# meudnaes/VoronoiRT

Hardware: AMD Instinct MI355X
Metric: formal-solve cell-updates/sec (higher is better)
Workload: dtype f64

## Files before the change

include/voronoirt.h:

```cpp
#ifndef VORONOIRT_H
#define VORONOIRT_H

#include <stdint.h>

#ifdef __cplusplus
extern "C" {
#endif

#define VRT_OK 0
#define VRT_EINVAL (-1)
#define VRT_EGRID (-2)
#define VRT_ENODEVICE (-3)
#define VRT_ENOMEM (-4)
#define VRT_EIO (-5)

typedef struct vrt_grid vrt_grid;
typedef struct vrt_plan vrt_plan;

#define VRT_ALPHA_SITE 0
#define VRT_ALPHA_SITE_LAM 1
#define VRT_ALPHA_ANGLE_SITE_LAM 2
#define VRT_ALPHA_ANGLE_NATIVE 3
#define VRT_ALPHA_SITE_LAM_NATIVE 4

// ... 25 lines not shown
                       int n_sweeps, vrt_plan **out);
void vrt_plan_destroy(vrt_plan *p);
int64_t vrt_plan_num_levels(const vrt_plan *p);
int64_t vrt_plan_num_nodes(const vrt_plan *p);
int vrt_plan_get_upwind(const vrt_plan *p, int64_t angle, int64_t *up, double *dots, double *w,
                        double *r);

int vrt_plan_execute(vrt_plan *p, int64_t nlam, int64_t ld, const double *S, const double *alpha,
                     int alpha_mode, const double *I0_up, const double *I0_down,
                     const double *weights, double *J, double *I_out);
int vrt_plan_execute_dev(vrt_plan *p, int64_t nlam, int64_t ld, const double *dS,
                         const double *dalpha, int alpha_mode, const double *dI0_up,
                         const double *dI0_down, const double *weights_host, double *dJ,
                         double *dI_out, void *stream);
int vrt_grid_get_storage_order(const vrt_grid *g, int dir, int64_t *out);
int64_t vrt_plan_native_alpha_count(const vrt_plan *p, int64_t nlam);
int vrt_plan_native_pair_block(const vrt_plan *p);
int vrt_plan_native_pair_block_f32(const vrt_plan *p);
int vrt_plan_alpha_to_native_dev(vrt_plan *p, int64_t nlam, int64_t ld, const double *dalpha,
                                 double *dalpha_native, void *stream);
int vrt_plan_alpha_to_native_dev_f32(vrt_plan *p, int64_t nlam, int64_t ld, const float *dalpha,
                                     float *dalpha_native, void *stream);

int64_t vrt_plan_native_plane_count(const vrt_plan *p, int64_t nlam);
int vrt_plan_to_native_dev(vrt_plan *p, int64_t nlam, int64_t ld, const double *d_in, double *d_up, double *d_down,
                           void *stream);
int vrt_plan_from_native_dev(vrt_plan *p, int dir, int64_t nlam, int64_t ld, const double *d_native, double *d_out,
                             void *stream);
int vrt_plan_j_from_native_dev(vrt_plan *p, int64_t nlam, int64_t ld, const double *dJ_up, const double *dJ_down,
                               double *dJ, void *stream);
int vrt_plan_execute_native_dev(vrt_plan *p, int64_t nlam, const double *dS_up, const double *dS_down,
                                const double *dalpha, int alpha_mode, const double *dI0_up, const double *dI0_down,
                                const double *weights_host, double *dJ_up, double *dJ_down, void *stream);
int vrt_plan_to_native_dev_f32(vrt_plan *p, int64_t nlam, int64_t ld, const float *d_in, float *d_up, float *d_down,
                               void *stream);
int vrt_plan_from_native_dev_f32(vrt_plan *p, int dir, int64_t nlam, int64_t ld, const float *d_native, float *d_out,
                                 void *stream);
int vrt_plan_j_from_native_dev_f32(vrt_plan *p, int64_t nlam, int64_t ld, const float *dJ_up, const float *dJ_down,
                                   float *dJ, void *stream);
int vrt_plan_execute_native_dev_f32(vrt_plan *p, int64_t nlam, const float *dS_up, const float *dS_down,
                                    const float *dalpha, int alpha_mode, const float *dI0_up, const float *dI0_down,
                                    const double *weights_host, float *dJ_up, float *dJ_down, void *stream);

int vrt_lambda_update_native_dev(vrt_grid *g, int64_t nlam, const double *dJ_up, const double *dJ_down,
                                 const double *dB_up, const double *deps, double *dS_up, double *dS_down,
                                 double *max_rel_change, void *stream);
int vrt_rates_populations_native_dev(vrt_grid *g, int64_t nlam, const double *lambda, const int64_t blocks[6],
                                     const double *dJ_up, const double *dJ_down, const double *planck2,
                                     double lambda0, double c0, const double *d_doppler_width, const double *d_gamma,
                                     double sigma_bb_const, const double *sigma_bf1, const double *sigma_bf2,
                                     const double *d_temperature, const double *d_lte_populations, double hc_over_kB,
                                     double pref_ij, double pref_ji, const double *d_C, const double *d_atom_density,
                                     double *d_R, double *d_populations, void *stream);

int vrt_plan_execute_dev_f32(vrt_plan *p, int64_t nlam, int64_t ld, const float *dS,
                             const float *dalpha, int alpha_mode, const float *dI0_up,
                             const float *dI0_down, const double *weights_host, float *dJ,
                             float *dI_out, void *stream);
int vrt_plan_last_sweep_timing(const vrt_plan *p, double *ms, int64_t *launches);
int vrt_plan_check(vrt_plan *p);
int vrt_plan_last_path(const vrt_plan *p);
int vrt_plan_set_option(vrt_plan *p, const char *name, const char *value);
int vrt_grid_set_option(vrt_grid *g, const char *name, const char *value);

typedef struct vrt_schedule vrt_schedule;
int vrt_schedule_build(const vrt_grid *g, int dir, const int64_t *up, int n_sweeps, vrt_schedule **out);
int64_t vrt_schedule_num_nodes(const vrt_schedule *s);
int64_t vrt_schedule_num_levels(const vrt_schedule *s);
int vrt_schedule_get(const vrt_schedule *s, int64_t *site, int32_t *zflags, int64_t *level_off);
void vrt_schedule_destroy(vrt_schedule *s);
int vrt_layer_schedule(const vrt_grid *g, int dir, const int64_t *up, int n_sweeps, uint32_t *vis,
                       int32_t *nlev, int64_t *n_visits);
int vrt_layer_sorted_slots(const vrt_grid *g, int dir, const uint32_t *vis, int64_t *store, int64_t *self);

typedef struct vrt_patch_schedule vrt_patch_schedule;
int vrt_patch_schedule_build(const vrt_grid *g, int dir, const int64_t *up, int n_sweeps, int own_target,
                             int entry_cap, vrt_patch_schedule **out, int64_t counts[6]);
int vrt_patch_schedule_get(const vrt_patch_schedule *s, int32_t *layer_patch_off, int32_t *patch_own_lo,
                           int32_t *patch_own_cnt, int32_t *patch_nlev, int64_t *patch_ent_off,
                           int32_t *entry_pos, uint32_t *entry_vis, uint32_t *entry_loc);
int vrt_patch_schedule_get_deps(const vrt_patch_schedule *s, int64_t *dep_off, int32_t *dep_list);
int vrt_patch_schedule_get_layers(const vrt_patch_schedule *s, uint32_t *vis, int32_t *nlev, int64_t *n_visits);
void vrt_patch_schedule_destroy(vrt_patch_schedule *s);

int vrt_delaunay_up(vrt_grid *g, const double k[3], const double *S, const double *I0,
                    int64_t nI0, const double *alpha, int n_sweeps, double *I_out);
int vrt_delaunay_down(vrt_grid *g, const double k[3], const double *S, const double *I0,
                      int64_t nI0, const double *alpha, int n_sweeps, double *I_out);

#define VRT_METRIC_EUCLIDEAN   0
#define VRT_METRIC_PERIODIC_XY 1
#define VRT_RASTER_NEAREST     1
#define VRT_RASTER_INV_DIST2   2
int vrt_grid_nearest(vrt_grid *g, int64_t nq, const double *q_zxy, int metric, int k, int64_t *idx, double *dist);
int vrt_grid_to_raster_dev(vrt_grid *g, int64_t nz, int64_t nx, int64_t ny, const double *z, const double *x,
                           const double *y, int metric, int mode, int64_t nf, int64_t ld, const double *d_fields,
                           double *d_raster, void *stream);
int vrt_raster_to_grid_dev(vrt_grid *g, int64_t nz, int64_t nx, int64_t ny, const double *z, const double *x,
                           const double *y, int64_t nf, const double *d_raster, int64_t ld, double *d_fields,
                           void *stream);
int vrt_grid_to_raster(vrt_grid *g, int64_t nz, int64_t nx, int64_t ny, const double *z, const double *x,
                       const double *y, int metric, int mode, int64_t nf, int64_t ld, const double *fields,
                       double *raster);
int vrt_raster_to_grid(vrt_grid *g, int64_t nz, int64_t nx, int64_t ny, const double *z, const double *x,
                       const double *y, int64_t nf, const double *raster, int64_t ld, double *fields);
int vrt_grid_raster_stats(const vrt_grid *g, double *nearest_ms, double *gather_ms, int64_t *queries,
                          int64_t *walk_steps, int64_t *fallbacks);

int vrt_sample_sites(int device, int64_t nz, int64_t nx, int64_t ny, const double *z, const double *x, const double *y,
                     const double *quantity, int64_t n_sites, uint64_t seed, int64_t batch, int64_t max_proposals,
                     double *pos_zxy, int64_t *proposals_used);
int vrt_sample_sites_dev(int device, int64_t nz, int64_t nx, int64_t ny, const double *z, const double *x,
                         const double *y, const double *d_quantity, int64_t n_sites, uint64_t seed, int64_t batch,
                         int64_t max_proposals, double *d_pos_zxy, int64_t *proposals_used, void *stream);

int vrt_lambda_update_dev(vrt_grid *g, int64_t nlam, int64_t ld, const double *dJ, const double *dB,
                          const double *deps, const double *dS_old, double *dS_new,
                          double *max_rel_change, void *stream);

int vrt_line_opacity_dev(vrt_plan *p, int64_t nlam, const double *lambda, double lambda0, double c0,
                         const double *d_velocity, const double *d_doppler_width, const double *d_gamma,
                         const double *d_line_strength, const double *d_alpha_cont, double *d_alpha_native,
                         void *stream);
int vrt_line_opacity_dev_f32(vrt_plan *p, int64_t nlam, const double *lambda, double lambda0, double c0,
                             const double *d_velocity, const double *d_doppler_width, const double *d_gamma,
                             const double *d_line_strength, const double *d_alpha_cont, float *d_alpha_native,
                             void *stream);

int vrt_plan_execute_line(vrt_plan *p, int64_t nlam, int64_t ld, const double *lambda, double lambda0, double c0,
                          const double *velocity, const double *doppler_width, const double *gamma,
                          const double *line_strength, const double *alpha_cont, const double *S, const double *I0_up,
                          const double *I0_down, const double *weights, double *J);

int vrt_line_terms_dev(vrt_grid *g, const double *d_gamma_static, const double *d_gamma_unsold,
                       const double *d_populations, double strength_const, double Bij, double Bji, double *d_gamma,
                       double *d_line_strength, void *stream);

typedef struct vrt_lambda vrt_lambda;
typedef struct vrt_line_case {
    int64_t nlam;
    const double *lambda;
    int64_t blocks[6];
    double lambda0, c0;
    const double *velocity;
    const double *doppler_width;
    const double *gamma_static;
    const double *gamma_unsold;
    const double *alpha_cont;
    const double *eps;
    const double *temperature;
    const double *atom_density;
    const double *B0;
    const double *lte_populations;
    const double *C;
    const double *planck2;
    const double *sigma_bf1, *sigma_bf2;
    double strength_const, Bij, Bji;
    double sigma_bb_const, hc_over_kB, pref_ij, pref_ji;
} vrt_line_case;
int vrt_lambda_create(vrt_plan *p, const vrt_line_case *lc, const double *weights, vrt_lambda **out);
int vrt_lambda_iterate(vrt_lambda *s, double *max_rel_change);
int vrt_lambda_get(vrt_lambda *s, double *J, double *S, double *populations, double *R, double *gamma);
void vrt_lambda_destroy(vrt_lambda *s);

typedef struct vrt_multi vrt_multi;
int vrt_multi_create(int n_devices, const int *devices, int64_t n, const double *pos_zxy, const int64_t *nbr, int64_t D1,
// ... 80 lines not shown
```

voronoirt_amd/_lib.py:

```python
from __future__ import annotations

import ctypes
import os

HERE = os.path.dirname(os.path.abspath(__file__))
LIB_PATH = os.path.join(HERE, "libvrt_hip.so")
if os.environ.get("VRT_LIB_PATH"):
    LIB_PATH = os.environ["VRT_LIB_PATH"]

c_i64 = ctypes.c_int64
c_dbl = ctypes.c_double
p_i64 = ctypes.POINTER(ctypes.c_int64)
p_i32 = ctypes.POINTER(ctypes.c_int32)
p_dbl = ctypes.POINTER(ctypes.c_double)
p_int = ctypes.POINTER(ctypes.c_int)
vp = ctypes.c_void_p

VRT_OK, VRT_EINVAL, VRT_EGRID, VRT_ENODEVICE, VRT_ENOMEM, VRT_EIO = 0, -1, -2, -3, -4, -5
ALPHA_SITE, ALPHA_SITE_LAM, ALPHA_ANGLE_SITE_LAM, ALPHA_ANGLE_NATIVE, ALPHA_SITE_LAM_NATIVE = 0, 1, 2, 3, 4
METRIC_EUCLIDEAN, METRIC_PERIODIC_XY = 0, 1
RASTER_NEAREST, RASTER_INV_DIST2 = 1, 2

class LineCaseStruct(ctypes.Structure):
    _fields_ = [("nlam", c_i64), ("lambda_", p_dbl), ("blocks", c_i64 * 6), ("lambda0", c_dbl), ("c0", c_dbl),
# ... 20 lines not shown
    "vrt_grid_num_layer_offsets": (c_i64, [vp, ctypes.c_int]),
    "vrt_grid_get_layers": (ctypes.c_int, [vp, ctypes.c_int, p_i64]),
    "vrt_grid_get_perm": (ctypes.c_int, [vp, ctypes.c_int, p_i64]),
    "vrt_grid_get_delaunay_lines": (ctypes.c_int, [vp, p_dbl]),
    "vrt_direction": (None, [c_dbl, c_dbl, p_dbl]),
    "vrt_plan_create": (ctypes.c_int, [vp, c_i64, p_dbl, ctypes.c_int, ctypes.POINTER(vp)]),
    "vrt_plan_create_ex": (ctypes.c_int, [vp, c_i64, p_dbl, p_int, ctypes.c_int,
                                          ctypes.POINTER(vp)]),
    "vrt_plan_destroy": (None, [vp]),
    "vrt_plan_num_levels": (c_i64, [vp]),
    "vrt_plan_num_nodes": (c_i64, [vp]),
    "vrt_plan_get_upwind": (ctypes.c_int, [vp, c_i64, p_i64, p_dbl, p_dbl, p_dbl]),
    "vrt_plan_execute": (ctypes.c_int, [vp, c_i64, c_i64, p_dbl, p_dbl, ctypes.c_int, p_dbl, p_dbl,
                                        p_dbl, p_dbl, p_dbl]),
    "vrt_plan_execute_dev": (ctypes.c_int, [vp, c_i64, c_i64, vp, vp, ctypes.c_int, vp, vp, p_dbl,
                                            vp, vp, vp]),
    "vrt_plan_execute_dev_f32": (ctypes.c_int, [vp, c_i64, c_i64, vp, vp, ctypes.c_int, vp, vp, p_dbl,
                                                vp, vp, vp]),
    "vrt_plan_native_plane_count": (c_i64, [vp, c_i64]),
    "vrt_plan_to_native_dev": (ctypes.c_int, [vp, c_i64, c_i64, vp, vp, vp, vp]),
    "vrt_plan_from_native_dev": (ctypes.c_int, [vp, ctypes.c_int, c_i64, c_i64, vp, vp, vp]),
    "vrt_plan_j_from_native_dev": (ctypes.c_int, [vp, c_i64, c_i64, vp, vp, vp, vp]),
    "vrt_plan_execute_native_dev": (ctypes.c_int, [vp, c_i64, vp, vp, vp, ctypes.c_int, vp, vp, p_dbl, vp, vp, vp]),
    "vrt_plan_to_native_dev_f32": (ctypes.c_int, [vp, c_i64, c_i64, vp, vp, vp, vp]),
    "vrt_plan_from_native_dev_f32": (ctypes.c_int, [vp, ctypes.c_int, c_i64, c_i64, vp, vp, vp]),
    "vrt_plan_j_from_native_dev_f32": (ctypes.c_int, [vp, c_i64, c_i64, vp, vp, vp, vp]),
    "vrt_plan_execute_native_dev_f32": (ctypes.c_int, [vp, c_i64, vp, vp, vp, ctypes.c_int, vp, vp, p_dbl, vp, vp, vp]),
    "vrt_plan_check": (ctypes.c_int, [vp]),
    "vrt_lambda_update_native_dev": (ctypes.c_int, [vp, c_i64, vp, vp, vp, vp, vp, vp, p_dbl, vp]),
    "vrt_rates_populations_native_dev": (ctypes.c_int, [vp, c_i64, p_dbl, p_i64, vp, vp, p_dbl, c_dbl, c_dbl, vp, vp,
                                                        c_dbl, p_dbl, p_dbl, vp, vp, c_dbl, c_dbl, c_dbl, vp, vp, vp,
                                                        vp, vp]),
    "vrt_grid_get_storage_order": (ctypes.c_int, [vp, ctypes.c_int, p_i64]),
    "vrt_plan_native_alpha_count": (c_i64, [vp, c_i64]),
    "vrt_plan_native_pair_block": (ctypes.c_int, [vp]),
    "vrt_plan_native_pair_block_f32": (ctypes.c_int, [vp]),
    "vrt_plan_alpha_to_native_dev": (ctypes.c_int, [vp, c_i64, c_i64, vp, vp, vp]),
    "vrt_line_opacity_dev": (ctypes.c_int, [vp, c_i64, p_dbl, c_dbl, c_dbl, vp, vp, vp, vp, vp, vp, vp]),
    "vrt_line_opacity_dev_f32": (ctypes.c_int, [vp, c_i64, p_dbl, c_dbl, c_dbl, vp, vp, vp, vp, vp, vp, vp]),
    "vrt_plan_alpha_to_native_dev_f32": (ctypes.c_int, [vp, c_i64, c_i64, vp, vp, vp]),
    "vrt_plan_execute_line": (ctypes.c_int, [vp, c_i64, c_i64, p_dbl, c_dbl, c_dbl, p_dbl, p_dbl, p_dbl, p_dbl, p_dbl,
                                             p_dbl, p_dbl, p_dbl, p_dbl, p_dbl]),
    "vrt_line_terms_dev": (ctypes.c_int, [vp, vp, vp, vp, c_dbl, c_dbl, c_dbl, vp, vp, vp]),
    "vrt_lambda_create": (ctypes.c_int, [vp, ctypes.POINTER(LineCaseStruct), p_dbl, ctypes.POINTER(vp)]),
    "vrt_lambda_iterate": (ctypes.c_int, [vp, p_dbl]),
    "vrt_lambda_get": (ctypes.c_int, [vp, p_dbl, p_dbl, p_dbl, p_dbl, p_dbl]),
    "vrt_lambda_destroy": (None, [vp]),
    "vrt_multi_create": (ctypes.c_int, [ctypes.c_int, p_int, c_i64, p_dbl, p_i64, c_i64, p_dbl, c_i64, p_dbl, p_int,
                                        ctypes.c_int, ctypes.POINTER(vp)]),
    "vrt_multi_execute": (ctypes.c_int, [vp, c_i64, c_i64, p_dbl, p_dbl, ctypes.c_int, p_dbl, p_dbl, p_dbl, p_dbl]),
    "vrt_multi_set_shard": (ctypes.c_int, [vp, ctypes.c_char_p]),
    "vrt_multi_last_shard": (ctypes.c_int, [vp]),
    "vrt_multi_uses_rccl": (ctypes.c_int, [vp]),
    "vrt_multi_destroy": (None, [vp]),
    "vrt_multi_execute_line": (ctypes.c_int, [vp, c_i64, c_i64, p_dbl, c_dbl, c_dbl, p_dbl, p_dbl, p_dbl, p_dbl, p_dbl, p_dbl,
                                              p_dbl, p_dbl, p_dbl, p_dbl]),
    "vrt_multi_lambda_create": (ctypes.c_int, [vp, ctypes.POINTER(LineCaseStruct), p_dbl, ctypes.POINTER(vp)]),
    "vrt_multi_lambda_iterate": (ctypes.c_int, [vp, p_dbl]),
    "vrt_multi_lambda_get": (ctypes.c_int, [vp, p_dbl, p_dbl, p_dbl, p_dbl, p_dbl]),
    "vrt_multi_lambda_destroy": (None, [vp]),
    "vrt_rates_populations_dev": (ctypes.c_int, [vp, c_i64, c_i64, p_dbl, p_i64, vp, p_dbl, c_dbl, c_dbl, vp, vp,
                                                 c_dbl, p_dbl, p_dbl, vp, vp, c_dbl, c_dbl, c_dbl, vp, vp, vp,
                                                 vp, vp]),
    "vrt_plan_last_sweep_timing": (ctypes.c_int, [vp, p_dbl, p_i64]),
    "vrt_plan_last_path": (ctypes.c_int, [vp]),
    "vrt_plan_set_option": (ctypes.c_int, [vp, ctypes.c_char_p, ctypes.c_char_p]),
    "vrt_grid_set_option": (ctypes.c_int, [vp, ctypes.c_char_p, ctypes.c_char_p]),
    "vrt_schedule_build": (ctypes.c_int, [vp, ctypes.c_int, p_i64, ctypes.c_int,
                                          ctypes.POINTER(vp)]),
    "vrt_schedule_num_nodes": (c_i64, [vp]),
    "vrt_schedule_num_levels": (c_i64, [vp]),
    "vrt_schedule_get": (ctypes.c_int, [vp, p_i64, p_i32, p_i64]),
    "vrt_schedule_destroy": (None, [vp]),
    "vrt_layer_schedule": (ctypes.c_int, [vp, ctypes.c_int, p_i64, ctypes.c_int,
                                          ctypes.POINTER(ctypes.c_uint32), p_i32, p_i64]),
    "vrt_layer_sorted_slots": (ctypes.c_int, [vp, ctypes.c_int, ctypes.POINTER(ctypes.c_uint32), p_i64, p_i64]),
    "vrt_patch_schedule_build": (ctypes.c_int, [vp, ctypes.c_int, p_i64, ctypes.c_int, ctypes.c_int, ctypes.c_int,
                                                ctypes.POINTER(vp), p_i64]),
    "vrt_patch_schedule_get": (ctypes.c_int, [vp, p_i32, p_i32, p_i32, p_i32, p_i64, p_i32,
                                              ctypes.POINTER(ctypes.c_uint32), ctypes.POINTER(ctypes.c_uint32)]),
    "vrt_patch_schedule_get_deps": (ctypes.c_int, [vp, p_i64, p_i32]),
    "vrt_patch_schedule_get_layers": (ctypes.c_int, [vp, ctypes.POINTER(ctypes.c_uint32), p_i32, p_i64]),
    "vrt_patch_schedule_destroy": (None, [vp]),
    "vrt_lambda_update_dev": (ctypes.c_int, [vp, c_i64, c_i64, vp, vp, vp, vp, vp, p_dbl, vp]),
    "vrt_short_characteristics": (ctypes.c_int, [c_i64, c_i64, c_i64, p_dbl, p_dbl, p_dbl, c_i64, p_dbl,
                                                 p_int, p_dbl, c_i64, p_dbl, c_i64, p_dbl, ctypes.c_int,
                                                 ctypes.c_int, p_dbl]),
    "vrt_regular_create": (ctypes.c_int, [c_i64, c_i64, c_i64, p_dbl, p_dbl, p_dbl, ctypes.c_int,
                                          ctypes.POINTER(vp)]),
    "vrt_regular_destroy": (None, [vp]),
    "vrt_regular_execute_dev": (ctypes.c_int, [vp, c_i64, p_dbl, p_int, vp, c_i64, vp, c_i64, c_i64, vp,
                                               ctypes.c_int, vp, vp]),
    "vrt_regular_last_solve_ms": (ctypes.c_int, [vp, p_dbl]),
    "vrt_regular_execute_line": (ctypes.c_int, [vp, c_i64, p_dbl, p_int, p_dbl, c_i64, p_dbl, c_dbl, c_dbl, p_dbl, p_dbl,
                                                p_dbl, p_dbl, p_dbl, p_dbl, p_dbl, ctypes.c_int, p_dbl]),
    "vrt_regular_lambda_create": (ctypes.c_int, [vp, c_i64, p_dbl, p_int, p_dbl, ctypes.POINTER(LineCaseStruct), ctypes.c_int,
                                                 ctypes.POINTER(vp)]),
    "vrt_regular_lambda_iterate": (ctypes.c_int, [vp, p_dbl]),
    "vrt_regular_lambda_get": (ctypes.c_int, [vp, p_dbl, p_dbl, p_dbl, p_dbl, p_dbl]),
    "vrt_regular_lambda_destroy": (None, [vp]),
    "vrt_synth_opacity_dev": (ctypes.c_int, [c_i64, c_i64, c_i64, p_dbl, c_i64, p_dbl, p_dbl, c_dbl, c_dbl, c_dbl, c_dbl,
                                             c_dbl, c_dbl, c_dbl, c_dbl, vp, vp, vp, vp, vp, vp, vp, vp, vp, vp]),
    "vrt_synth_opacity": (ctypes.c_int, [ctypes.c_int, c_i64, c_i64, c_i64, p_dbl, c_i64, p_dbl, p_dbl, c_dbl, c_dbl,
                                         c_dbl, c_dbl, c_dbl, c_dbl, c_dbl, c_dbl, p_dbl, p_dbl, p_dbl, p_dbl, p_dbl,
                                         p_dbl, p_dbl, p_dbl, p_dbl]),
    "vrt_regular_emergent_dev": (ctypes.c_int, [vp, p_dbl, c_i64, vp, vp, ctypes.c_int, vp, vp]),
    "vrt_top_intensity": (ctypes.c_int, [c_i64, c_i64, c_i64, p_dbl, p_dbl, p_dbl, p_dbl, c_i64, p_dbl, p_dbl,
                                         ctypes.c_int, ctypes.c_int, p_dbl]),
    "vrt_tau_unity_dev": (ctypes.c_int, [c_i64, c_i64, c_i64, p_dbl, p_dbl, p_dbl, p_dbl, c_i64, vp, vp, vp]),
    "vrt_tau_unity": (ctypes.c_int, [c_i64, c_i64, c_i64, p_dbl, p_dbl, p_dbl, p_dbl, c_i64, p_dbl, ctypes.c_int,
                                     p_dbl]),
    "vrt_grid_nearest": (ctypes.c_int, [vp, c_i64, p_dbl, ctypes.c_int, ctypes.c_int, p_i64, p_dbl]),
    "vrt_grid_to_raster_dev": (ctypes.c_int, [vp, c_i64, c_i64, c_i64, p_dbl, p_dbl, p_dbl, ctypes.c_int, ctypes.c_int,
                                              c_i64, c_i64, vp, vp, vp]),
    "vrt_raster_to_grid_dev": (ctypes.c_int, [vp, c_i64, c_i64, c_i64, p_dbl, p_dbl, p_dbl, c_i64, vp, c_i64, vp, vp]),
    "vrt_grid_to_raster": (ctypes.c_int, [vp, c_i64, c_i64, c_i64, p_dbl, p_dbl, p_dbl, ctypes.c_int, ctypes.c_int,
                                          c_i64, c_i64, p_dbl, p_dbl]),
    "vrt_raster_to_grid": (ctypes.c_int, [vp, c_i64, c_i64, c_i64, p_dbl, p_dbl, p_dbl, c_i64, p_dbl, c_i64, p_dbl]),
    "vrt_grid_raster_stats": (ctypes.c_int, [vp, p_dbl, p_dbl, p_i64, p_i64, p_i64]),
    "vrt_sample_sites": (ctypes.c_int, [ctypes.c_int, c_i64, c_i64, c_i64, p_dbl, p_dbl, p_dbl, p_dbl, c_i64,
                                        ctypes.c_uint64, c_i64, c_i64, p_dbl, p_i64]),
    "vrt_sample_sites_dev": (ctypes.c_int, [ctypes.c_int, c_i64, c_i64, c_i64, p_dbl, p_dbl, p_dbl, vp, c_i64,
                                            ctypes.c_uint64, c_i64, c_i64, vp, p_i64, vp]),
    "vrt_delaunay_up": (ctypes.c_int, [vp, p_dbl, p_dbl, p_dbl, c_i64, p_dbl, ctypes.c_int, p_dbl]),
    "vrt_delaunay_down": (ctypes.c_int, [vp, p_dbl, p_dbl, p_dbl, c_i64, p_dbl, ctypes.c_int, p_dbl]),
}


class VrtError(RuntimeError):
    def __init__(self, code: int, message: str):
        super().__init__(f"libvrt_hip error {code}: {message}")
        self.code = code
        self.message = message


_lib = None


def load() -> ctypes.CDLL:
    global _lib
    if _lib is not None:
        return _lib
    if not os.path.exists(LIB_PATH):
        raise ImportError(
            f"{LIB_PATH} is missing: build it with `python -m voronoirt_amd.build` "
            "(hipcc --offload-arch=gfx950).  voronoirt_amd has no CPU fallback.")
    if os.environ.get("VRT_NO_TORCH") != "1":
        try:
            import torch
        except Exception:
            pass
    lib = ctypes.CDLL(LIB_PATH)
    for name, (res, args) in PROTOTYPES.items():
        fn = getattr(lib, name)
        fn.restype = res
        fn.argtypes = args
    _lib = lib
    return lib


def check(rc: int) -> None:
    if rc != 0:
        msg = load().vrt_last_error()
        raise VrtError(rc, msg.decode() if msg else "")
```

voronoirt_amd/csrc/vrt_api.cpp:

```cpp
#include <algorithm>
#include <atomic>
#include <chrono>
#include <cmath>
#include <cstdio>
#include <cstdlib>
#include <cstring>
#include <memory>
#include <new>
#include <thread>

#include "vrt_internal.h"

namespace vrt {

static thread_local std::string g_err;

void set_error(const std::string &msg) { g_err = msg; }
int fail(int code, const std::string &msg)
{
    g_err = msg;
    return code;
}

void tuning_from_env(Tuning &t)
{
    static const char *names[] = {"VRT_PATH", "VRT_STEP_K", "VRT_STEP_SINGLE", "VRT_STEP_PAIRS", "VRT_STEP_XCD",
                                  "VRT_STEP_STREAMS", "VRT_STEP_LEVEL_MAP", "VRT_STEP_GROUP_DIR", "VRT_TILE_WIDE",
                                  "VRT_TILE_PRE", "VRT_PATCH_K", "VRT_PATCH_NT", "VRT_PATCH_OWN",
                                  "VRT_PATCH_Q", "VRT_PATCH_TARGET", "VRT_PATCH_SPLIT", "VRT_PAIR_BLOCK", "VRT_PATCH_QUAD", "VRT_PATCH_LEAN", "VRT_PATCH_CHAIN", "VRT_CHAIN_PAIRS", "VRT_CHAIN_SPIN", "VRT_CHAIN_DATAFLAG", "VRT_CHAIN_STATIC", "VRT_LAMBDA_NATIVE", "VRT_DEBUG_FLAGS", "VRT_DEBUG_SKIP_LEVELS",
                                  "VRT_TILE_DEBUG"};
    for (const char *nm : names) {
        const char *e = std::getenv(nm);
        if (e && *e && tuning_set(t, nm, e, false) != VRT_OK) {
            static std::mutex mu;
            static std::vector<std::string> said;
            std::lock_guard<std::mutex> lock(mu);
            if (std::find(said.begin(), said.end(), std::string(nm)) == said.end()) {
                said.push_back(nm);
                std::fprintf(stderr, "[libvrt_hip] ignoring %s=%s: %s\n", nm, e, g_err.c_str());
            }
        }
    }
}

int tuning_set(Tuning &t, const char *name, const char *value, bool created)
{
    if (!name || !value) return fail(VRT_EINVAL, "NULL option name or value");
    const std::string nm(name), v(value);
    if (nm == "VRT_PATH") {
        static const char *paths[] = {"auto", "levels", "tiles", "steps", "patches"};
        for (int i = 0; i < 5; i++)
            if (v == paths[i]) { t.path = i; return VRT_OK; }
        if (v.empty()) { t.path = 0; return VRT_OK; }
        return fail(VRT_EINVAL, "VRT_PATH must be auto, levels, tiles, steps or patches");
    }
    char *end = nullptr;
    const long x = std::strtol(value, &end, 10);
    if (end == value || *end != 0) return fail(VRT_EINVAL, "option " + nm + " needs an integer value");
    struct { const char *name; int *field; long lo, hi; bool creation_only; } tab[] = {
        {"VRT_STEP_K", &t.step_K, 0, 18, false}, {"VRT_STEP_SINGLE", &t.step_single, 0, 1, false},
        {"VRT_STEP_PAIRS", &t.step_pairs, 0, 64, false}, {"VRT_STEP_XCD", &t.step_xcd, 0, 2, false},
        {"VRT_STEP_STREAMS", &t.step_streams, 1, 4, false}, {"VRT_STEP_LEVEL_MAP", &t.step_level_map, 0, 1, false},
        {"VRT_STEP_GROUP_DIR", &t.step_group_dir, 0, 1, false}, {"VRT_TILE_WIDE", &t.tile_wide, 0, 1, false},
        {"VRT_TILE_PRE", &t.tile_pre, 0, 1, false},
        {"VRT_PATCH_K", &t.patch_K, 1, 8, true}, {"VRT_PATCH_NT", &t.patch_NT, 64, 1024, true},
        {"VRT_PATCH_OWN", &t.patch_own, 0, 65535, true}, {"VRT_PATCH_Q", &t.patch_Q, 1, 4, false},
        {"VRT_PATCH_TARGET", &t.patch_target, 0, 1 << 20, false}, {"VRT_PATCH_SPLIT", &t.patch_split, 0, 4096, false}, {"VRT_PAIR_BLOCK", &t.pair_block, 1, 16, true},
        {"VRT_PATCH_QUAD", &t.patch_quad, 0, 1, true}, {"VRT_PATCH_LEAN", &t.patch_lean, 0, 1, false},
        {"VRT_PATCH_CHAIN", &t.patch_chain, 0, 2, false}, {"VRT_CHAIN_PAIRS", &t.chain_pairs, 1, 256, false},
        {"VRT_CHAIN_SPIN", &t.chain_spin, 1, 1 << 20, false}, {"VRT_CHAIN_DATAFLAG", &t.chain_dataflag, 0, 2, false},
        {"VRT_LAMBDA_NATIVE", &t.lambda_native, 0, 1, false}, {"VRT_CHAIN_STATIC", &t.chain_static, 0, 1, false}, {"VRT_DEBUG_FLAGS", &t.debug_flags, 0, 1 << 20, false},
        {"VRT_DEBUG_SKIP_LEVELS", &t.debug_skip_levels, 0, 1, false}, {"VRT_TILE_DEBUG", &t.tile_debug, 0, 1, false},
    };
    for (auto &o : tab)
        if (nm == o.name) {
            if (o.creation_only && created)
                return fail(VRT_EINVAL, "option " + nm + " shapes what plan creation builds: preset it in the environment");
            if (x < o.lo || x > o.hi) return fail(VRT_EINVAL, "option " + nm + " out of range");
            *o.field = (int)x;
            return VRT_OK;
        }
    return fail(VRT_EINVAL, "unknown option " + nm);
}

int use_device(int device)
{
    if (device < 0)
        return fail(VRT_ENODEVICE, "host-only grid handle (device < 0): no compute without a HIP device");
    int cnt = 0;
    hipError_t e = hipGetDeviceCount(&cnt);
    if (e != hipSuccess || cnt <= 0)
        return fail(VRT_ENODEVICE, "no HIP device available (libvrt_hip has no CPU fallback)");
    if (device < 0 || device >= cnt) return fail(VRT_EINVAL, "device ordinal out of range");
    VRT_HIP_TRY(hipSetDevice(device));
    (void)hipGetLastError();
    return VRT_OK;
}

int use_current_device()
{
    int cnt = 0;
    if (hipGetDeviceCount(&cnt) != hipSuccess || cnt <= 0)
        return fail(VRT_ENODEVICE, "no HIP device available (libvrt_hip has no CPU fallback)");
    (void)hipGetLastError();
    return VRT_OK;
}

static void free_grid(vrt_grid *g)
{
    if (!g) return;
    for (PlanCacheEntry *c : g->cache) {
        vrt_plan_destroy(c->plan);
        delete c;
    }
    g->cache.clear();
    raster_locator_free(g);
    dev_free(g->d_pos);
    dev_free(g->d_rowptr);
    dev_free(g->d_col);
    dev_free(g->d_lz);
    dev_free(g->d_lx);
    dev_free(g->d_ly);
    dev_free(g->up.d_order);
    dev_free(g->down.d_order);
    dev_free(g->up.d_rank);
    dev_free(g->down.d_rank);
    dev_free(g->up.d_lay);
    dev_free(g->down.d_lay);
    dev_free(g->d_scalars);
    dev_free(g->d_small);
    if (g->small_ev) (void)hipEventDestroy(g->small_ev);
    if (g->small_copy_ev) (void)hipEventDestroy(g->small_copy_ev);
    if (g->h_small) (void)hipHostFree(g->h_small);
    dev_free(g->up.d_store);
    dev_free(g->down.d_store);
    dev_free(g->up.d_srank);
    dev_free(g->down.d_srank);
    if (g->stream) (void)hipStreamDestroy(g->stream);
    delete g;
}

static int upload_grid(vrt_grid *g)
{
    const int64_t n = g->n;
    const size_t nnz = g->col.size();
    int rc;
    if ((rc = dev_alloc(&g->d_pos, (size_t)3 * n))) return rc;
    if ((rc = dev_alloc(&g->d_rowptr, (size_t)n + 1))) return rc;
    if ((rc = dev_alloc(&g->d_col, nnz))) return rc;
    if ((rc = dev_alloc(&g->d_lz, nnz))) return rc;
// ... 9 lines not shown
        std::vector<int32_t> order((size_t)n);
        for (int64_t i = 0; i < n; i++) order[(size_t)i] = (int32_t)(dir.perm[(size_t)i] - 1);
        if ((rc = dev_alloc(&dir.d_order, (size_t)n))) return rc;
        VRT_HIP_TRY(hipMemcpy(dir.d_order, order.data(), sizeof(int32_t) * n, hipMemcpyHostToDevice));
        std::vector<int32_t> rank((size_t)n);
        for (int64_t i = 0; i < n; i++) rank[(size_t)order[(size_t)i]] = (int32_t)i;
        if ((rc = dev_alloc(&dir.d_rank, (size_t)n))) return rc;
        VRT_HIP_TRY(hipMemcpy(dir.d_rank, rank.data(), sizeof(int32_t) * n, hipMemcpyHostToDevice));
        std::vector<int32_t> srank((size_t)n);
        for (int64_t i = 0; i < n; i++) srank[(size_t)dir.store[(size_t)i]] = (int32_t)i;
        if ((rc = dev_alloc(&dir.d_store, (size_t)n))) return rc;
        if ((rc = dev_alloc(&dir.d_srank, (size_t)n))) return rc;
        VRT_HIP_TRY(hipMemcpy(dir.d_store, dir.store.data(), sizeof(int32_t) * n, hipMemcpyHostToDevice));
        VRT_HIP_TRY(hipMemcpy(dir.d_srank, srank.data(), sizeof(int32_t) * n, hipMemcpyHostToDevice));
        std::vector<int32_t> lay(dir.reduced.size());
        for (size_t j = 0; j < lay.size(); j++) lay[j] = (int32_t)(dir.reduced[j] - 1);
        if ((rc = dev_alloc(&dir.d_lay, lay.size()))) return rc;
        VRT_HIP_TRY(hipMemcpy(dir.d_lay, lay.data(), sizeof(int32_t) * lay.size(), hipMemcpyHostToDevice));
    }
    if ((rc = launch_delaunay_lines(g))) return rc;
    VRT_HIP_TRY(hipStreamSynchronize(g->stream));
    return VRT_OK;
}

static int grid_create_impl(int64_t n, const double *pos, const int64_t *nbr, int64_t D1,
                            const double bounds[6], int device, vrt_grid **out)
{
    if (!out) return fail(VRT_EINVAL, "out is NULL");
    *out = nullptr;
    if (!pos || !nbr || !bounds) return fail(VRT_EINVAL, "NULL argument");
    int rc = device >= 0 ? use_device(device) : VRT_OK;
    if (rc) return rc;
    vrt_grid *g = new (std::nothrow) vrt_grid();
    if (!g) return fail(VRT_ENOMEM, "out of host memory");
    g->device = device;
    rc = build_grid_host(g, n, pos, nbr, D1, bounds);
    if (!rc && device >= 0) rc = upload_grid(g);
    if (rc) {
        free_grid(g);
        return rc;
    }
    *out = g;
    return VRT_OK;
}

static const Direction &direction_of(const vrt_grid *g, int dir) { return dir > 0 ? g->up : g->down; }

static void free_plan(vrt_plan *p)
{
    if (!p) return;
    dev_free(p->d_up1);
    dev_free(p->d_up2);
    dev_free(p->d_d1);
    dev_free(p->d_d2);
    dev_free(p->d_w1);
    dev_free(p->d_w2);
    dev_free(p->d_r1);
    dev_free(p->d_r2);
    dev_free(p->d_node_site);
    dev_free(p->d_node_meta);
    dev_free(p->d_node_u1);
    dev_free(p->d_node_u2);
    dev_free(p->d_angles_up);
    dev_free(p->d_angles_down);
    dev_free(p->d_I);
    for (int i = 0; i < 6; i++) dev_free(p->d_stage[i]);
    dev_free(p->t_u1); dev_free(p->t_u2);
    dev_free(p->t_w1); dev_free(p->t_w2); dev_free(p->t_r1); dev_free(p->t_r2);
    dev_free(p->t_vis);
    dev_free(p->t_loc);
    dev_free(p->t_self);
    dev_free(p->t_vis_s);
    dev_free(p->t_loc_s);
    dev_free(p->t_gpos);
    dev_free(p->t_rank_s);
    dev_free(p->t_loc_ss);
    dev_free(p->t_code_ss);
    dev_free(p->d_nlev); dev_free(p->d_angle_dir); dev_free(p->d_task_map);
    for (int d = 0; d < 2; d++) { dev_free(p->ws_S[d]); dev_free(p->ws_A[d]); dev_free(p->ws_J[d]); }
    dev_free(p->ws_AA);
    for (int i = 0; i < 2; i++) dev_free(p->ws_cg[i]);
    dev_free(p->d_step_angles);
    dev_free(p->d_level_map);
    dev_free(p->d_patch_work);
    dev_free(p->d_chain_items); dev_free(p->d_chain_deps); dev_free(p->d_chain_progress); dev_free(p->d_chain_ctrl);
    for (auto &cs : p->chain_cache) { dev_free(cs.items); dev_free(cs.deps); }
    p->chain_cache.clear();
    if (p->h_chain_status) { (void)hipHostFree(p->h_chain_status); p->h_chain_status = nullptr; }
    if (p->d_chain_dev) { (void)hipFree(p->d_chain_dev); p->d_chain_dev = nullptr; }
    if (p->h_chain_dev_pinned) { (void)hipHostFree(p->h_chain_dev_pinned); p->h_chain_dev_pinned = nullptr; }
    if (p->chain_dev_ev) (void)hipEventDestroy(p->chain_dev_ev);
    dev_free(p->e_pos); dev_free(p->e_u1); dev_free(p->e_u2); dev_free(p->e_vis); dev_free(p->e_loc);
    dev_free(p->e_w1); dev_free(p->e_w2); dev_free(p->e_r1); dev_free(p->e_r2);
    if (p->step_fork) (void)hipEventDestroy(p->step_fork);
    for (int i = 0; i < 4; i++) {
        if (p->step_join[i]) (void)hipEventDestroy(p->step_join[i]);
        if (p->step_stream[i]) (void)hipStreamDestroy(p->step_stream[i]);
    }
    for (CopyLane &l : p->copy_lanes) {
        for (int b = 0; b < 2; b++) {
            if (l.pin[b]) (void)hipHostFree(l.pin[b]);
            if (l.ev[b]) (void)hipEventDestroy(l.ev[b]);
        }
        if (l.st) (void)hipStreamDestroy(l.st);
    }
    if (p->copy_done) (void)hipEventDestroy(p->copy_done);
    if (p->ev0) (void)hipEventDestroy(p->ev0);
    if (p->ev1) (void)hipEventDestroy(p->ev1);
    delete p;
}

static int ensure_level_schedule(vrt_plan *p)
{
    if (p->level_ready) return VRT_OK;
    vrt_grid *g = p->g;
    const int64_t n = g->n;
    const int A = p->A;
    const int n_sweeps = p->n_sweeps;
    std::vector<AngleSchedule> sched((size_t)A);
    {
        unsigned hw = std::thread::hardware_concurrency();
        int nthr = (int)std::min<unsigned>(hw ? hw : 4, 16);
        nthr = std::max(1, std::min(nthr, std::max(A, 1)));
        if (!run_workers(nthr, [&](int t) {
                for (int a = t; a < A; a += nthr) {
                    const bool up = p->dir_of_active[(size_t)a] > 0;
                    build_angle_schedule(up ? g->up : g->down, up, n, n_sweeps,
                                         p->h_up1.data() + (size_t)a * n, p->h_up2.data() + (size_t)a * n,
                                         sched[(size_t)a]);
                }
            }))
            return fail(VRT_ENOMEM, "out of host memory while building the level schedule");
    }
    int64_t max_levels = 0, total = 0;
    for (int a = 0; a < A; a++) {
        if (sched[(size_t)a].bad_site >= 0) return fail(VRT_EGRID, "site without an upwind neighbour");
        max_levels = std::max<int64_t>(max_levels, (int64_t)sched[(size_t)a].level_off.size() - 1);
        total += (int64_t)sched[(size_t)a].site.size();
    }
    std::vector<int32_t> srank_up((size_t)n);
    for (int64_t i = 0; i < n; i++) srank_up[(size_t)g->up.store[(size_t)i]] = (int32_t)i;
    std::vector<uint32_t> node_site((size_t)total), node_meta((size_t)total);
    std::vector<int32_t> node_u1((size_t)total), node_u2((size_t)total);
    p->level_off.assign((size_t)max_levels + 1, 0);
    int64_t at = 0;
    for (int64_t t = 0; t < max_levels; t++) {
        p->level_off[(size_t)t] = at;
        for (int a = 0; a < A; a++) {
            const AngleSchedule &s = sched[(size_t)a];
            if (t + 1 >= (int64_t)s.level_off.size()) continue;
            const int64_t x0 = s.level_off[(size_t)t], x1 = s.level_off[(size_t)t + 1];
            std::vector<std::pair<int32_t, int64_t>> keyed((size_t)(x1 - x0));
            for (int64_t x = x0; x < x1; x++)
                keyed[(size_t)(x - x0)] = {srank_up[(size_t)s.site[(size_t)x]], x};
            std::sort(keyed.begin(), keyed.end());
            for (const auto &kv : keyed) {
                const int64_t x = kv.second;
                node_site[(size_t)at] = s.site[(size_t)x];
                node_meta[(size_t)at] = (uint32_t)a | ((uint32_t)s.zflags[(size_t)x] << 8);
                node_u1[(size_t)at] = p->h_up1[(size_t)a * (size_t)n + s.site[(size_t)x]];
                node_u2[(size_t)at] = p->h_up2[(size_t)a * (size_t)n + s.site[(size_t)x]];
                at++;
            }
        }
    }
    p->level_off[(size_t)max_levels] = at;
    p->n_nodes = total;
// ... 773 lines not shown
        return VRT_OK;
    });
}

struct vrt_patch_schedule {
    vrt::PatchSchedule s;
    vrt::LayerSchedule layers;
};

int vrt_patch_schedule_build(const vrt_grid *g, int dir, const int64_t *up, int n_sweeps, int own_target,
                             int entry_cap, vrt_patch_schedule **out, int64_t counts[6])
{
    if (!g || !up || !out || !counts) return fail(VRT_EINVAL, "NULL argument");
    if (n_sweeps < 1 || own_target < 1 || entry_cap < 1 || entry_cap > 65535)
        return fail(VRT_EINVAL, "need n_sweeps >= 1, own_target >= 1 and 1 <= entry_cap <= 65535");
    *out = nullptr;
    return guarded([&] {
        const int64_t n = g->n;
        std::vector<int32_t> u1((size_t)n), u2((size_t)n);
        for (int64_t i = 0; i < n; i++) {
            const int64_t a = up[2 * i], b = up[2 * i + 1];
            if (a > n || b > n) return fail(VRT_EINVAL, "upwind id out of range");
            u1[(size_t)i] = a >= 1 ? (int32_t)(a - 1) : kNoUpwind;
            u2[(size_t)i] = b >= 1 ? (int32_t)(b - 1) : kNoUpwind;
        }
        std::unique_ptr<vrt_patch_schedule> ps(new vrt_patch_schedule());
        int threads = (int)std::max(1u, std::min(8u, std::thread::hardware_concurrency()));
        if (const char *e = std::getenv("VRT_HOST_THREADS")) threads = std::max(1, std::min(64, std::atoi(e)));
        build_patch_schedule(direction_of(g, dir), dir > 0, n, n_sweeps, u1.data(), u2.data(), own_target, entry_cap,
                             ps->s, threads, &ps->layers);
        if (ps->s.bad_site >= 0)
            return fail(VRT_EGRID, "site " + std::to_string(ps->s.bad_site + 1) + " has no upwind neighbour");
        if (!ps->s.ok) return fail(VRT_EINVAL, "schedule does not fit the packed patch encoding");
        counts[0] = (int64_t)ps->s.patch_own_lo.size();
        counts[1] = (int64_t)ps->s.entry_pos.size();
        counts[2] = ps->s.n_visits;
        counts[3] = ps->s.n_live;
        counts[4] = ps->s.max_entries;
        counts[5] = (int64_t)ps->s.layer_patch_off.size();
        *out = ps.release();
        return VRT_OK;
    });
}

int vrt_patch_schedule_get(const vrt_patch_schedule *s, int32_t *layer_patch_off, int32_t *patch_own_lo,
                           int32_t *patch_own_cnt, int32_t *patch_nlev, int64_t *patch_ent_off,
                           int32_t *entry_pos, uint32_t *entry_vis, uint32_t *entry_loc)
{
    if (!s) return fail(VRT_EINVAL, "NULL schedule");
    const PatchSchedule &p = s->s;
    if (layer_patch_off) std::copy(p.layer_patch_off.begin(), p.layer_patch_off.end(), layer_patch_off);
    if (patch_own_lo) std::copy(p.patch_own_lo.begin(), p.patch_own_lo.end(), patch_own_lo);
    if (patch_own_cnt) std::copy(p.patch_own_cnt.begin(), p.patch_own_cnt.end(), patch_own_cnt);
    if (patch_nlev) std::copy(p.patch_nlev.begin(), p.patch_nlev.end(), patch_nlev);
    if (patch_ent_off) std::copy(p.patch_ent_off.begin(), p.patch_ent_off.end(), patch_ent_off);
    if (entry_pos) std::copy(p.entry_pos.begin(), p.entry_pos.end(), entry_pos);
    if (entry_vis) std::copy(p.entry_vis.begin(), p.entry_vis.end(), entry_vis);
    if (entry_loc) std::copy(p.entry_loc.begin(), p.entry_loc.end(), entry_loc);
    return VRT_OK;
}

int vrt_patch_schedule_get_deps(const vrt_patch_schedule *s, int64_t *dep_off, int32_t *dep_list)
{
    if (!s) return fail(VRT_EINVAL, "NULL schedule");
    const PatchSchedule &p = s->s;
    if (dep_off) std::copy(p.dep_off.begin(), p.dep_off.end(), dep_off);
    if (dep_list) std::copy(p.dep_list.begin(), p.dep_list.end(), dep_list);
    return VRT_OK;
}

int vrt_patch_schedule_get_layers(const vrt_patch_schedule *s, uint32_t *vis, int32_t *nlev, int64_t *n_visits)
{
    if (!s) return fail(VRT_EINVAL, "NULL schedule");
    const LayerSchedule &ls = s->layers;
    if (!ls.ok) return fail(VRT_EINVAL, "schedule does not fit the packed layer-tile encoding");
    if (vis) std::copy(ls.vis.begin(), ls.vis.end(), vis);
    if (nlev) std::copy(ls.nlev.begin(), ls.nlev.end(), nlev);
    if (n_visits) *n_visits = ls.n_visits;
    return VRT_OK;
}

void vrt_patch_schedule_destroy(vrt_patch_schedule *s) { delete s; }

int vrt_grid_get_storage_order(const vrt_grid *g, int dir, int64_t *out)
{
    if (!g || !out) return fail(VRT_EINVAL, "NULL argument");
    const Direction &d = direction_of(g, dir);
    for (int64_t i = 0; i < g->n; i++) out[i] = (int64_t)d.store[(size_t)i] + 1;
    return VRT_OK;
}

int vrt_plan_native_pair_block(const vrt_plan *p) { return p ? 1 << native_lg(p, false) : 0; }
int vrt_plan_native_pair_block_f32(const vrt_plan *p) { return p ? 1 << native_lg(p, true) : 0; }

int64_t vrt_plan_native_alpha_count(const vrt_plan *p, int64_t nlam)
{
    if (!p || nlam < 1) return 0;
    return (int64_t)p->A * ((nlam + 1) / 2 * 2) * p->g->n;
}

static int alpha_native_call(vrt_plan *p, int64_t nlam, int64_t ld, const void *dalpha, void *dalpha_native, void *stream,
                             bool f32)
{
    return guarded([&] {
        if (!p || !dalpha || !dalpha_native) return fail(VRT_EINVAL, "NULL argument");
        if (nlam < 1 || ld < nlam) return fail(VRT_EINVAL, "need nlam >= 1 and ld >= nlam");
        if (p->A != (int)p->n_angles_user)
            return fail(VRT_EINVAL, "per-angle alpha needs every angle active (no θ = 90 direction)");
        std::lock_guard<std::mutex> lock(p->mu);
        int rc = use_device(p->g->device);
        return rc ? rc : alpha_to_native(p, nlam, ld, dalpha, dalpha_native, (hipStream_t)stream, f32);
    });
}

int vrt_plan_alpha_to_native_dev(vrt_plan *p, int64_t nlam, int64_t ld, const double *dalpha,
                                 double *dalpha_native, void *stream)
{
    return alpha_native_call(p, nlam, ld, dalpha, dalpha_native, stream, false);
}

int vrt_plan_alpha_to_native_dev_f32(vrt_plan *p, int64_t nlam, int64_t ld, const float *dalpha, float *dalpha_native,
                                     void *stream)
{
    return alpha_native_call(p, nlam, ld, dalpha, dalpha_native, stream, true);
}

int vrt_plan_execute_dev(vrt_plan *p, int64_t nlam, int64_t ld, const double *dS,
                         const double *dalpha, int alpha_mode, const double *dI0_up,
                         const double *dI0_down, const double *weights_host, double *dJ,
                         double *dI_out, void *stream)
{
    return execute_call(p, caller_args(nlam, ld, dS, dalpha, alpha_mode, dI0_up, dI0_down, weights_host, dJ, dI_out,
                                       (hipStream_t)stream, false));
}

int64_t vrt_plan_native_plane_count(const vrt_plan *p, int64_t nlam)
{
    if (!p || nlam < 1) return 0;
    return ((nlam + 1) / 2 * 2) * p->g->n;
}

int vrt_plan_to_native_dev(vrt_plan *p, int64_t nlam, int64_t ld, const double *d_in, double *d_up, double *d_down, void *stream)
{
    return native_call(p, nlam, ld, d_in && (d_up || d_down), false,
                       [&] { return planes_to_native(p, nlam, ld, d_in, d_up, d_down, (hipStream_t)stream); });
}

int vrt_plan_from_native_dev(vrt_plan *p, int dir, int64_t nlam, int64_t ld, const double *d_native, double *d_out, void *stream)
{
    return native_call(p, nlam, ld, d_native && d_out, false,
                       [&] { return plane_from_native(p, dir > 0 ? 0 : 1, nlam, ld, d_native, d_out, (hipStream_t)stream); });
}

int vrt_plan_j_from_native_dev(vrt_plan *p, int64_t nlam, int64_t ld, const double *dJ_up, const double *dJ_down, double *dJ,
                               void *stream)
{
    return native_call(p, nlam, ld, dJ && (dJ_up || dJ_down), false,
                       [&] { return J_from_native(p, nlam, ld, dJ_up, dJ_down, dJ, (hipStream_t)stream); });
}

int vrt_plan_execute_native_dev(vrt_plan *p, int64_t nlam, const double *dS_up, const double *dS_down, const double *dalpha,
                                int alpha_mode, const double *dI0_up, const double *dI0_down, const double *weights_host,
                                double *dJ_up, double *dJ_down, void *stream)
{
    return execute_call(p, native_args(nlam, dS_up, dS_down, dalpha, alpha_mode, dI0_up, dI0_down, weights_host, dJ_up,
                                       dJ_down, (hipStream_t)stream, false));
// ... 384 lines not shown
```

voronoirt_amd/csrc/vrt_internal.h:

```cpp
#pragma once

#include <hip/hip_runtime.h>

#include <algorithm>
#include <cstdint>
#include <mutex>
#include <new>
#include <string>
#include <thread>
#include <vector>

#include "voronoirt.h"

namespace vrt {

void set_error(const std::string &msg);
int fail(int code, const std::string &msg);

#define VRT_HIP_TRY(expr)                                                                  \
    do {                                                                                   \
        hipError_t _e = (expr);                                                            \
        if (_e != hipSuccess)                                                              \
            return ::vrt::fail(VRT_ENODEVICE, std::string(#expr) + ": " + hipGetErrorString(_e)); \
    } while (0)
// ... 65 lines not shown
    ~DevBuf() { dev_free(p); }
    int alloc(size_t count) { dev_free(p); return dev_alloc(&p, count); }
    operator T *() const { return p; }
};

template <typename Body>
inline bool run_workers(int count, Body body)
{
    std::vector<char> threw((size_t)std::max(count, 1), 0);
    auto guarded = [&](int t) {
        try {
            body(t);
        } catch (...) {
            threw[(size_t)t] = 1;
        }
    };
    std::vector<std::thread> pool;
    try {
        pool.reserve((size_t)std::max(count, 1));
    } catch (...) {
    }
    for (int t = 0; t < count; t++) {
        try {
            pool.emplace_back(guarded, t);
        } catch (...) {
            guarded(t);
        }
    }
    for (auto &th : pool) th.join();
    for (int t = 0; t < count; t++)
        if (threw[(size_t)t]) return false;
    return true;
}

constexpr int kMaxAngles = 64;
constexpr int64_t kMaxGuess = 70;
constexpr int32_t kNoUpwind = -1;

struct Direction {
    std::vector<int32_t> layer_of;
    std::vector<int64_t> perm;
    std::vector<int64_t> reduced;
    int64_t n1 = 0;
    int32_t *d_order = nullptr;
    int32_t *d_rank = nullptr;
    int32_t *d_lay = nullptr;
    std::vector<int32_t> store;
    int32_t *d_store = nullptr;
    int32_t *d_srank = nullptr;
};

struct PlanCacheEntry;

struct CopyLane {
    hipStream_t st = nullptr;
    void *pin[2] = {nullptr, nullptr};
    hipEvent_t ev[2] = {nullptr, nullptr};
};
constexpr size_t kCopyChunk = (size_t)8 << 20;

struct Tuning {
    int path = 0;
    int step_K = 0;
    int step_single = 0;
    int step_pairs = 0;
    int step_xcd = 2;
    int step_streams = 2;
    int step_level_map = 1;
    int step_group_dir = 1;
    int tile_wide = 1;
    int tile_pre = 1;
    int patch_K = 1, patch_NT = 512;
    int patch_own = 0;
    int patch_Q = 1;
    int pair_block = 1;
    int patch_quad = 1;
    int patch_lean = 1;
    int patch_chain = 2;
    int chain_pairs = 9;
    int chain_spin = 2048;
    int chain_dataflag = 2;
    int patch_split = 0;
    int patch_target = 0;
    int chain_static = 1;
    int lambda_native = 1;
    int debug_flags = 0, debug_skip_levels = 0, tile_debug = 0;
};
void tuning_from_env(Tuning &t);
int tuning_set(Tuning &t, const char *name, const char *value, bool created);

struct ExecArgs {
    int64_t nlam = 0, ld = 0;
    const void *S = nullptr;
    const void *S_nat[2] = {nullptr, nullptr};
    const void *alpha = nullptr;
    int alpha_mode = 0;
    const void *I0[2] = {nullptr, nullptr};
    const double *weights = nullptr;
    void *J = nullptr;
    void *J_nat[2] = {nullptr, nullptr};
    void *I_out = nullptr;
    bool native = false;
    bool f32 = false;
    hipStream_t st = nullptr;
    bool wants_J() const { return native ? J_nat[0] != nullptr : J != nullptr; }
};
inline ExecArgs caller_args(int64_t nlam, int64_t ld, const void *S, const void *alpha, int alpha_mode, const void *I0_up,
                            const void *I0_down, const double *weights, void *J, void *I_out, hipStream_t st, bool f32)
{
    ExecArgs x;
    x.nlam = nlam; x.ld = ld;
    x.S = S;
    x.alpha = alpha; x.alpha_mode = alpha_mode;
    x.I0[0] = I0_up; x.I0[1] = I0_down;
    x.weights = weights;
    x.J = J; x.I_out = I_out;
    x.f32 = f32;
    x.st = st;
    return x;
}
inline ExecArgs native_args(int64_t nlam, const void *S_up, const void *S_down, const void *alpha, int alpha_mode,
                            const void *I0_up, const void *I0_down, const double *weights, void *J_up, void *J_down,
                            hipStream_t st, bool f32)
{
    ExecArgs x = caller_args(nlam, (nlam + 1) / 2 * 2, nullptr, alpha, alpha_mode, I0_up, I0_down, weights, nullptr, nullptr,
                             st, f32);
    x.S_nat[0] = S_up; x.S_nat[1] = S_down;
    x.J_nat[0] = J_up; x.J_nat[1] = J_down;
    x.native = true;
    return x;
}

}

namespace vrt {
struct RasterLocator;
void raster_locator_free(vrt_grid *g);
}

struct vrt_grid {
    int device = 0;
    int64_t n = 0;
    int64_t D = 0;
    double bounds[6] = {0, 0, 0, 0, 0, 0};
    std::vector<double> pos;
    std::vector<int32_t> rowptr;
    std::vector<int32_t> col;
    vrt::Direction up, down;
    double *d_pos = nullptr;
    int32_t *d_rowptr = nullptr;
    int32_t *d_col = nullptr;
    double *d_lz = nullptr, *d_lx = nullptr, *d_ly = nullptr;
    hipStream_t stream = nullptr;
    unsigned long long *d_scalars = nullptr;
    double *d_small = nullptr;
    size_t small_cap = 0;
    double *h_small = nullptr;
    hipEvent_t small_ev = nullptr;
    bool small_ev_valid = false;
    hipEvent_t small_copy_ev = nullptr;
    bool small_copy_valid = false;
    std::vector<std::pair<std::string, std::string>> options;
    std::mutex mu;
    std::vector<vrt::PlanCacheEntry *> cache;
    vrt::RasterLocator *locator = nullptr;
    int64_t nearest_cells = 0;
// ... 16 lines not shown
    uint32_t *d_node_meta = nullptr;
    int32_t *d_node_u1 = nullptr, *d_node_u2 = nullptr;
    std::vector<int64_t> level_off;
    bool level_ready = false;
    std::vector<int32_t> h_up1, h_up2;
    int64_t n_nodes = 0;
    int32_t *d_angles_up = nullptr, *d_angles_down = nullptr;
    int n_up = 0, n_down = 0;
    std::vector<int64_t> skip_site;
    double *d_I = nullptr;
    size_t I_cap = 0;
    int64_t I_ld = 0;
    double *d_stage[6] = {nullptr, nullptr, nullptr, nullptr, nullptr, nullptr};
    size_t stage_cap[6] = {0, 0, 0, 0, 0, 0};
    bool tile_ok = false;
    bool step_tables_ready = false;
    int tile_K = 8;
    int tile_max_layers = 0;
    int64_t tile_max_layer_size = 0;
    int64_t tile_visits = 0;
    int32_t *t_u1 = nullptr, *t_u2 = nullptr;
    double *t_w1 = nullptr, *t_w2 = nullptr, *t_r1 = nullptr, *t_r2 = nullptr;
    uint32_t *t_vis = nullptr, *t_loc = nullptr;
    int32_t *t_self = nullptr;
    uint32_t *t_vis_s = nullptr, *t_loc_s = nullptr;
    uint32_t *t_gpos = nullptr;
    int32_t *t_rank_s = nullptr;
    uint32_t *t_loc_ss = nullptr;
    uint32_t *t_code_ss = nullptr;
    int32_t *d_nlev = nullptr, *d_angle_dir = nullptr;
    std::vector<int64_t> angle_visits;
    std::vector<int32_t> h_task_map;
    int32_t *d_task_map = nullptr;
    size_t task_map_cap = 0;
    int task_map_nlam = -1;
    double *ws_S[2] = {nullptr, nullptr}, *ws_A[2] = {nullptr, nullptr}, *ws_J[2] = {nullptr, nullptr};
    size_t ws_S_cap[2] = {0, 0}, ws_A_cap[2] = {0, 0}, ws_J_cap[2] = {0, 0};
    double *ws_AA = nullptr;
    size_t ws_AA_cap = 0;
    double *ws_cg[2] = {nullptr, nullptr};
    size_t ws_cg_cap[2] = {0, 0};
    int step_groups = 0;
    int32_t *d_step_angles = nullptr;
    std::vector<int> step_group_off;
    std::vector<double> angle_mean_levels;
    int32_t *d_level_map = nullptr;
    std::vector<int> level_map_off;
    int level_map_units = 0, level_map_groups = 0;
    std::vector<int32_t> h_step_angles;
    bool patch_ok = false;
    int lg_pair_block = 0;
    int patch_cap = 0, patch_K = 0, patch_NT = 0;
    int64_t n_patches = 0, n_patch_entries = 0, n_patch_visits = 0;
    std::vector<int32_t> h_patch_first;
    std::vector<int4> h_patch_rec;
    int32_t *e_pos = nullptr, *e_u1 = nullptr, *e_u2 = nullptr;
    uint32_t *e_vis = nullptr, *e_loc = nullptr;
    double *e_w1 = nullptr, *e_w2 = nullptr, *e_r1 = nullptr, *e_r2 = nullptr;
    std::vector<int2> h_patch_rec2;
    std::vector<int64_t> h_patch_dep_off;
    std::vector<int32_t> h_patch_deps;
    int4 *d_chain_items = nullptr;
    int32_t *d_chain_deps = nullptr;
    uint32_t *d_chain_progress = nullptr, *d_chain_ctrl = nullptr;
    uint32_t *h_chain_status = nullptr, *d_chain_status = nullptr;
    void *d_chain_dev = nullptr, *h_chain_dev_pinned = nullptr;
    std::vector<char> h_chain_dev;
    hipEvent_t chain_dev_ev = nullptr;
    bool chain_dev_ev_valid = false;
    size_t chain_progress_cap = 0;
    bool chain_progress_fresh = false;
    int chain_q_off[9] = {0, 0, 0, 0, 0, 0, 0, 0, 0};
    int chain_npair = -1, chain_lgB = -1, chain_nsplit = -1, chain_reduce = -1;
    int64_t chain_items = 0;
    struct ChainSet {
        int npair = -1, lgB = -1, nsplit = -1, reduce = -1;
        int4 *items = nullptr;
        int32_t *deps = nullptr;
        int q_off[9] = {0, 0, 0, 0, 0, 0, 0, 0, 0};
        int64_t n_items = 0;
    };
    std::vector<ChainSet> chain_cache;
    uint32_t chain_epoch = 0;
    int4 *d_patch_work = nullptr;
    std::vector<int64_t> patch_work_off;
    int patch_work_groups = 0;
    hipStream_t step_stream[4] = {nullptr, nullptr, nullptr, nullptr};
    hipEvent_t step_fork = nullptr, step_join[4] = {nullptr, nullptr, nullptr, nullptr};
    int last_path = 0;
    hipEvent_t ev0 = nullptr, ev1 = nullptr;
    bool ev_valid = false;
    std::vector<vrt::CopyLane> copy_lanes;
    hipEvent_t copy_done = nullptr;
    int64_t last_launches = 0;
    std::mutex mu;
};

namespace vrt {

struct PlanCacheEntry {
    double k[3];
    int n_sweeps;
    vrt_plan *plan;
    int users;
};

int parse_neighbour_file(const char *path, int64_t n, std::vector<int64_t> &matrix, int64_t &D1);
int build_grid_host(vrt_grid *g, int64_t n, const double *pos, const int64_t *nbr, int64_t D1,
                    const double bounds[6]);

int tessellate_host(int64_t n, const double *pos, const double bounds[6], int64_t D1, int64_t *nbr_out,
                    int64_t *max_count, int nthreads);

struct AngleSchedule {
    std::vector<uint32_t> site;
    std::vector<uint8_t> zflags;
    std::vector<int64_t> level_off;
    int64_t bad_site = -1;
};
void build_angle_schedule(const Direction &dir, bool ascending, int64_t n, int n_sweeps,
                          const int32_t *up1, const int32_t *up2, AngleSchedule &out);
struct LayerSchedule {
    std::vector<uint32_t> vis;
    std::vector<int32_t> nlev;
    int64_t n_visits = 0;
    int64_t max_layer_size = 0;
    int64_t bad_site = -1;
    bool ok = false;
};
void build_layer_schedule(const Direction &dir, bool ascending, int64_t n, int n_sweeps,
                          const int32_t *up1, const int32_t *up2, LayerSchedule &out);
void build_sorted_slots(const Direction &dir, int64_t n, const std::vector<uint32_t> &vis_site,
                        std::vector<int32_t> &self);
struct PatchSchedule {
    std::vector<int32_t> layer_patch_off;
    std::vector<int32_t> patch_own_lo;
    std::vector<int32_t> patch_own_cnt;
    std::vector<int32_t> patch_nlev;
    std::vector<int64_t> patch_ent_off;
    std::vector<int32_t> entry_pos;
    std::vector<uint32_t> entry_vis;
    std::vector<uint32_t> entry_loc;
    std::vector<int64_t> dep_off;
    std::vector<int32_t> dep_list;
    int64_t n_visits = 0;
    int64_t n_live = 0;
    int64_t max_entries = 0;
    int64_t bad_site = -1;
    bool ok = false;
};
void build_patch_schedule(const Direction &dir, bool ascending, int64_t n, int n_sweeps, const int32_t *up1,
                          const int32_t *up2, int own_target, int entry_cap, PatchSchedule &out, int threads = 1,
                          LayerSchedule *layers = nullptr);

int launch_delaunay_lines(vrt_grid *g);
int launch_upwind_table(vrt_plan *p, int a);
struct SweepArgs {
    int64_t n, nlam, ldS, ldA, ldI;
    const void *S, *alpha;
    int alpha_mode;
    void *I;
    bool f32 = false;
};
int launch_boundary(vrt_plan *p, const SweepArgs &sa, const void *dI0_up, const void *dI0_down,
                    hipStream_t st);
int launch_sweep_levels(vrt_plan *p, const SweepArgs &sa, hipStream_t st, int64_t *launches);
int launch_reduce_J(vrt_plan *p, const SweepArgs &sa, const double *weights_active, void *dJ,
                    int64_t ldJ, hipStream_t st);
int launch_copy_I_out(vrt_plan *p, const SweepArgs &sa, void *dI_out, int64_t ldO, hipStream_t st);

int launch_axpy(size_t count, const double *d_src, double *d_dst, hipStream_t st);
int launch_gather_rows(int64_t rows, int64_t nlam, int64_t ld, const int32_t *d_order, const double *d_src, double *d_dst,
                       hipStream_t st);
int launch_lambda_update(int64_t n, int64_t nlam, int64_t ld, const double *dJ, const double *dB,
                         const double *deps, const double *dS_old, double *dS_new,
                         unsigned long long *d_result, hipStream_t st);
int launch_lambda_update_native(vrt_grid *g, int64_t nlam, const double *dJ_up, const double *dJ_down, const double *dB_up,
                                const double *deps, double *dS_up, double *dS_down, unsigned long long *d_result, hipStream_t st);

int launch_line_opacity(vrt_plan *p, int64_t nlam, const double *d_lambda, double lambda0, double c0,
                        const double *d_velocity, const double *d_doppler, const double *d_gamma,
                        const double *d_strength, const double *d_alpha_cont, void *d_out, hipStream_t st,
                        bool f32_out = false);
int launch_line_terms(int64_t n, const double *d_gamma_static, const double *d_gamma_unsold, const double *d_pops,
                      double strength_const, double Bij, double Bji, double *d_gamma, double *d_strength, hipStream_t st);
int launch_rates_populations(vrt_grid *g, int64_t nlam, int64_t ld, const int64_t blocks[6],
                             const double *d_small, const double *dJ, double lambda0, double c0,
                             const double *d_doppler, const double *d_gamma, double sigma_bb_const,
                             const double *d_temperature, const double *d_lte, double hc_over_kB,
                             double pref_ij, double pref_ji, const double *d_C, const double *d_atom_density,
                             double *d_R, double *d_populations, hipStream_t st,
                             const double *dJ_up = nullptr, const double *dJ_down = nullptr);
int launch_rates_populations(int64_t n, int64_t nlam, int64_t ld, const int64_t blocks[6], const double *d_small,
                             const double *dJ, double lambda0, double c0, const double *d_doppler, const double *d_gamma,
                             double sigma_bb_const, const double *d_temperature, const double *d_lte, double hc_over_kB,
                             double pref_ij, double pref_ji, const double *d_C, const double *d_atom_density, double *d_R,
                             double *d_populations, hipStream_t st);

int launch_rates_partial(vrt_grid *g, int64_t nlam, int64_t l0, int64_t l1, int64_t ld, const int64_t blocks[6],
                         const double *d_small, const double *dJ, double lambda0, double c0, const double *d_doppler,
                         const double *d_gamma, double sigma_bb_const, const double *d_temperature, const double *d_lte,
                         double hc_over_kB, double pref_ij, double pref_ji, double *d_shares, hipStream_t st,
                         const double *dJ_up = nullptr, const double *dJ_down = nullptr);
int launch_populations_from_shares(vrt_grid *g, const double *d_shares, const double *d_C, const double *d_atom_density,
                                   double *d_R, double *d_populations, hipStream_t st);

int execute_locked(vrt_plan *p, const ExecArgs &x);

int ensure_step_tables(vrt_plan *p);
int launch_permute_table(vrt_plan *p, int a, const uint32_t *d_vis_site);
int launch_sorted_tables(vrt_plan *p, int a);
int launch_gpos(vrt_plan *p, int a);
inline int native_lg(const vrt_plan *p, bool f32)
{
    if (!p->patch_ok) return 0;
    return f32 && p->tune.patch_quad != 0 && p->patch_K == 1 ? std::max(p->lg_pair_block, 1) : p->lg_pair_block;
}
int alpha_to_native(vrt_plan *p, int64_t nlam, int64_t ld, const void *dalpha, void *out, hipStream_t st, bool f32);
int native_planes_ok(const vrt_plan *p, bool f32 = false);
int planes_to_native_f32(vrt_plan *p, int64_t nlam, int64_t ld, const float *din, float *out_up, float *out_down, hipStream_t st);
int plane_from_native_f32(vrt_plan *p, int dir_index, int64_t nlam, int64_t ld, const float *din, float *dout, hipStream_t st);
int J_from_native_f32(vrt_plan *p, int64_t nlam, int64_t ld, const float *dJ_up, const float *dJ_down, float *dJ, hipStream_t st);
int planes_to_native(vrt_plan *p, int64_t nlam, int64_t ld, const double *din, double *out_up, double *out_down, hipStream_t st);
int plane_from_native(vrt_plan *p, int dir_index, int64_t nlam, int64_t ld, const double *din, double *dout, hipStream_t st);
int J_from_native(vrt_plan *p, int64_t nlam, int64_t ld, const double *dJ_up, const double *dJ_down, double *dJ, hipStream_t st);
int execute_layers(vrt_plan *p, const ExecArgs &x, int path);
int64_t steps_max_layer(bool f32);

struct TileArgs;
struct PatchReduce;
bool patch_shape_exists(int K, int Q, int NT);
int launch_patch_entries(vrt_plan *p, int a, int64_t first, int64_t count);
int ensure_patch_work(vrt_plan *p, int G, const std::vector<int32_t> &group_angles, const std::vector<int> &group_off);
int launch_patch_layer(vrt_plan *p, const TileArgs &ta, int npair, int layer, int group, int Q, hipStream_t st,
                       bool f32, const PatchReduce *reduce);
bool patch_chain_possible(const vrt_plan *p, int npair, bool f32);
bool patch_chain_dataflag(const vrt_plan *p, int npair, bool f32);
int launch_patch_chain(vrt_plan *p, const TileArgs &ta, int npair, hipStream_t st, bool f32, const PatchReduce *reduce,
                       bool dataflag, bool ctrl_zeroed = false);
int chain_ctrl_words();
int patch_chain_check(vrt_plan *p);

}
```

voronoirt_amd/csrc/vrt_layers.hip:

```cpp
#include <hip/hip_runtime.h>

#include <algorithm>
#include <cmath>
#include <cstdio>
#include <cstdlib>
#include <cstring>

#include "vrt_device.h"
#include "vrt_internal.h"

#include "vrt_layout_kernels.h"
#include "vrt_step_kernels.h"
#include "vrt_tile_kernels.h"

namespace vrt {

static int build_task_map(vrt_plan *p, int nlam, hipStream_t st)
{
    const int A = p->A;
    if (p->task_map_nlam == nlam && p->d_task_map) return VRT_OK;
    const int ntask = A * nlam;
    struct Group { int a, l0, l1; double cost; };
    std::vector<Group> groups;
    const int halves = nlam >= 2 ? 2 : 1;
// ... 86 lines not shown
int plane_from_native_f32(vrt_plan *p, int dir_index, int64_t nlam, int64_t ld, const float *din, float *dout, hipStream_t st)
{
    vrt_grid *g = p->g;
    const int64_t n = g->n;
    const dim3 tgrid((unsigned)((n + 63) / 64), (unsigned)((nlam + 63) / 64));
    const Direction &dir = dir_index == 0 ? g->up : g->down;
    hipLaunchKernelGGL(k_from_sweep_order<float>, tgrid, dim3(256), 0, st, n, (int)nlam, ld, 2 << native_lg(p, true), dir.d_store, din, dout);
    VRT_HIP_TRY(hipGetLastError());
    return VRT_OK;
}
int J_from_native_f32(vrt_plan *p, int64_t nlam, int64_t ld, const float *dJ_up, const float *dJ_down, float *dJ, hipStream_t st)
{
    vrt_grid *g = p->g;
    const int64_t n = g->n;
    const dim3 tgrid((unsigned)((n + 63) / 64), (unsigned)((nlam + 63) / 64));
    hipLaunchKernelGGL(k_combine_J<float>, tgrid, dim3(256), 0, st, n, (int)nlam, ld, 2 << native_lg(p, true), g->up.d_store, g->down.d_srank, dJ_up, dJ_down, dJ);
    VRT_HIP_TRY(hipGetLastError());
    return VRT_OK;
}

int planes_to_native(vrt_plan *p, int64_t nlam, int64_t ld, const double *din, double *out_up, double *out_down, hipStream_t st)
{
    vrt_grid *g = p->g;
    const int64_t n = g->n;
    const dim3 tgrid((unsigned)((n + 63) / 64), (unsigned)((nlam + 63) / 64));
    for (int d = 0; d < 2; d++) {
        double *out = d == 0 ? out_up : out_down;
        if (!out) continue;
        const Direction &dir = d == 0 ? g->up : g->down;
        hipLaunchKernelGGL(k_to_sweep_order<double>, tgrid, dim3(256), 0, st, n, (int)nlam, ld, 2, dir.d_store, din, out,
                           (const double *)nullptr, (double *)nullptr);
    }
    VRT_HIP_TRY(hipGetLastError());
    return VRT_OK;
}

int plane_from_native(vrt_plan *p, int dir_index, int64_t nlam, int64_t ld, const double *din, double *dout, hipStream_t st)
{
    vrt_grid *g = p->g;
    const int64_t n = g->n;
    const dim3 tgrid((unsigned)((n + 63) / 64), (unsigned)((nlam + 63) / 64));
    const Direction &dir = dir_index == 0 ? g->up : g->down;
    hipLaunchKernelGGL(k_from_sweep_order<double>, tgrid, dim3(256), 0, st, n, (int)nlam, ld, 2, dir.d_store, din, dout);
    VRT_HIP_TRY(hipGetLastError());
    return VRT_OK;
}

int J_from_native(vrt_plan *p, int64_t nlam, int64_t ld, const double *dJ_up, const double *dJ_down, double *dJ, hipStream_t st)
{
    vrt_grid *g = p->g;
    const int64_t n = g->n;
    const dim3 tgrid((unsigned)((n + 63) / 64), (unsigned)((nlam + 63) / 64));
    hipLaunchKernelGGL(k_combine_J<double>, tgrid, dim3(256), 0, st, n, (int)nlam, ld, 2, g->up.d_store, g->down.d_srank, dJ_up, dJ_down, dJ);
    VRT_HIP_TRY(hipGetLastError());
    return VRT_OK;
}

static int ensure_step_streams(vrt_plan *p, int G)
{
    if (p->step_groups == G && p->d_step_angles) return VRT_OK;
    const int A = p->A;
    std::vector<int32_t> order((size_t)A);
    for (int a = 0; a < A; a++) order[(size_t)a] = a;
    std::stable_sort(order.begin(), order.end(), [&](int32_t x, int32_t y) {
        return p->angle_visits[(size_t)x] > p->angle_visits[(size_t)y];
    });
    std::vector<int32_t> list;
    p->step_group_off.assign((size_t)G + 1, 0);
    const bool by_dir = G == 2 && p->n_up > 0 && std::abs(p->n_up - p->n_down) <= 1 &&
                        p->tune.step_group_dir != 0;
    for (int gi = 0; gi < G; gi++) {
        p->step_group_off[(size_t)gi] = (int)list.size();
        if (by_dir) {
            for (int j = 0; j < A; j++)
                if ((p->dir_of_active[(size_t)order[(size_t)j]] > 0) == (gi == 0)) list.push_back(order[(size_t)j]);
        } else
        for (int j = gi; j < A; j += G) list.push_back(order[(size_t)j]);
    }
    p->step_group_off[(size_t)G] = (int)list.size();
    int rc;
    if (!p->d_step_angles && (rc = dev_alloc(&p->d_step_angles, (size_t)A))) return rc;
    VRT_HIP_TRY(hipMemcpy(p->d_step_angles, list.data(), sizeof(int32_t) * list.size(), hipMemcpyHostToDevice));
    p->h_step_angles = list;
    dev_free(p->d_patch_work);
    if (!p->step_fork) VRT_HIP_TRY(hipEventCreateWithFlags(&p->step_fork, hipEventDisableTiming));
    for (int gi = 0; gi < 4; gi++) {
        if (gi >= 1 && gi < G && !p->step_stream[gi]) {
            VRT_HIP_TRY(hipStreamCreateWithFlags(&p->step_stream[gi], hipStreamNonBlocking));
            VRT_HIP_TRY(hipEventCreateWithFlags(&p->step_join[gi], hipEventDisableTiming));
        }
    }
    p->step_groups = G;
    return VRT_OK;
}

static int build_level_map(vrt_plan *p, int G, int units)
{
    if (p->d_level_map && p->level_map_groups == G && p->level_map_units == units) return VRT_OK;
    dev_free(p->d_level_map);
    double mean_all = 0.0;
    for (double v : p->angle_mean_levels) mean_all += v;
    mean_all = p->angle_mean_levels.empty() ? 1.0 : std::max(1.0, mean_all / (double)p->angle_mean_levels.size());
    std::vector<int32_t> h_angles((size_t)p->A);
    VRT_HIP_TRY(hipMemcpy(h_angles.data(), p->d_step_angles, sizeof(int32_t) * (size_t)p->A, hipMemcpyDeviceToHost));
    std::vector<int32_t> map;
    p->level_map_off.assign((size_t)G + 1, 0);
    for (int gi = 0; gi < G; gi++) {
        p->level_map_off[(size_t)gi] = (int)map.size();
        const int j0 = p->step_group_off[(size_t)gi], n_list = p->step_group_off[(size_t)gi + 1] - j0;
        const int ntask = n_list * units;
        if (ntask == 0) continue;
        std::vector<double> w((size_t)n_list);
        double W = 0.0;
        for (int j = 0; j < n_list; j++) {
            const int a = h_angles[(size_t)(j0 + j)];
            const double lv = (size_t)a < p->angle_mean_levels.size() ? p->angle_mean_levels[(size_t)a] : mean_all;
            w[(size_t)j] = 1.7 * mean_all + lv;
            W += w[(size_t)j] * units;
        }
        std::vector<std::vector<int32_t>> runs(8);
        double cum = 0.0;
        for (int t = 0; t < ntask; t++) {
            const double wt = w[(size_t)(t / units)];
            const int x = std::min(7, (int)((cum + 0.5 * wt) * 8.0 / W));
            runs[(size_t)x].push_back(t);
            cum += wt;
        }
        size_t per = 0;
        for (const auto &r : runs) per = std::max(per, r.size());
        for (size_t j = 0; j < per; j++)
            for (int x = 0; x < 8; x++) map.push_back(j < runs[(size_t)x].size() ? runs[(size_t)x][j] : -1);
    }
    p->level_map_off[(size_t)G] = (int)map.size();
    if (int rc = dev_alloc(&p->d_level_map, map.size())) return rc;
    VRT_HIP_TRY(hipMemcpy(p->d_level_map, map.data(), sizeof(int32_t) * map.size(), hipMemcpyHostToDevice));
    p->level_map_groups = G;
    p->level_map_units = units;
    return VRT_OK;
}

constexpr int kSingleMaxK64 = 12, kSingleMaxK32 = 18;

template <typename T, int K>
static void launch_levels1(dim3 grid, size_t lds, hipStream_t sg, const StepArgs &sa)
{
    hipLaunchKernelGGL((k_step_levels1<T, K>), grid, dim3(1024), lds, sg, sa);
}

template <typename T>
static void launch_levels1_K(int K, dim3 grid, size_t lds, hipStream_t sg, const StepArgs &sa)
{
    switch ((K + 1) / 2 * 2) {
    case 2: launch_levels1<T, 2>(grid, lds, sg, sa); break;
    case 4: launch_levels1<T, 4>(grid, lds, sg, sa); break;
    case 6: launch_levels1<T, 6>(grid, lds, sg, sa); break;
    case 8: launch_levels1<T, 8>(grid, lds, sg, sa); break;
    case 10: launch_levels1<T, 10>(grid, lds, sg, sa); break;
    case 12: launch_levels1<T, 12>(grid, lds, sg, sa); break;
    default:
        if (sizeof(T) == 4) {
            switch ((K + 1) / 2 * 2) {
            case 14: launch_levels1<float, 14>(grid, lds, sg, sa); break;
            case 16: launch_levels1<float, 16>(grid, lds, sg, sa); break;
            default: launch_levels1<float, 18>(grid, lds, sg, sa); break;
            }
        }
        break;
// ... 566 lines not shown
```

voronoirt_amd/csrc/vrt_patch.hip:

```cpp
#include <hip/hip_runtime.h>

#include <algorithm>
#include <cmath>
#include <cstdio>
#include <cstdlib>
#include <cstring>
#include <type_traits>

#include "vrt_device.h"
#include "vrt_internal.h"

namespace vrt {

enum : int {
    kDiagNoLevels = 1, kDiagCentreGathers = 2, kDiagNoWeights = 4, kDiagNoStores = 8, kDiagNoGatherI = 16, kDiagNoGatherAlpha = 32,
    kDiagNoGatherS = 64, kDiagNoReduce = 128, kDiagNoWait = 256, kDiagPlainLoadI = 512, kDiagPlainStoreI = 1024, kDiagNoPairLoop = 2048,
};
__host__ __device__ __forceinline__ constexpr bool diag(int dbg, int flag) { return kDiag && (dbg & flag) != 0; }

struct PatchArgs {
    TileArgs ta;
    int npair;
    int layer;
    int ngrp;
    int nsplit, Q;
    int lgB;
    int stride;
    int cap;
    int quad;
    int lean;
    int dbg;
    PatchReduce red;
    const int4 *wrec;
    const int32_t *e_pos, *e_u1, *e_u2;
    const uint32_t *e_vis, *e_loc;
    const double *e_w1, *e_w2, *e_r1, *e_r2;
};

__global__ void __launch_bounds__(256)
k_patch_entries(int64_t count, const int32_t *__restrict__ e_pos, const int32_t *__restrict__ t_u1,
                const int32_t *__restrict__ t_u2, const double *__restrict__ t_w1, const double *__restrict__ t_w2,
                const double *__restrict__ t_r1, const double *__restrict__ t_r2, int32_t *__restrict__ e_u1,
                int32_t *__restrict__ e_u2, double *__restrict__ e_w1, double *__restrict__ e_w2,
                double *__restrict__ e_r1, double *__restrict__ e_r2)
{
    const int64_t e = (int64_t)blockIdx.x * blockDim.x + threadIdx.x;
    if (e >= count) return;
    const int p = e_pos[e];
    e_u1[e] = t_u1[p]; e_u2[e] = t_u2[p];
    e_w1[e] = t_w1[p]; e_w2[e] = t_w2[p];
    e_r1[e] = t_r1[p]; e_r2[e] = t_r2[p];
}

int launch_patch_entries(vrt_plan *p, int a, int64_t first, int64_t count)
{
    if (count <= 0) return VRT_OK;
    const size_t o = (size_t)a * (size_t)p->g->n;
    hipLaunchKernelGGL(k_patch_entries, dim3((unsigned)((count + 255) / 256)), dim3(256), 0, p->g->stream, count,
                       p->e_pos + first, p->t_u1 + o, p->t_u2 + o, p->t_w1 + o, p->t_w2 + o, p->t_r1 + o,
                       p->t_r2 + o, p->e_u1 + first, p->e_u2 + first, p->e_w1 + first, p->e_w2 + first,
                       p->e_r1 + first, p->e_r2 + first);
    VRT_HIP_TRY(hipGetLastError());
    return VRT_OK;
}

__device__ __forceinline__ double exp_neg10(double x) { return exp_neg_tab(x); }

template <int MODE>
__device__ __forceinline__ void lin_weights_fma(double dtau, double &a, double &b, double &e)
{
    double rc = __builtin_amdgcn_rcp(dtau);
    rc = fma(fma(-dtau, rc, 1.0), rc, rc);
    double e_thin = 0.0, a_thin = 0.0, b_thin = 0.0;
    if (MODE != 1) {
        e_thin = fma(dtau, fma(0.5, dtau, -1.0), 1.0);
        a_thin = dtau * fma(dtau, -1.0 / 3.0, 0.5);
        b_thin = dtau * fma(dtau, -1.0 / 6.0, 0.5);
    }
    const bool thin = dtau < 5e-4;
    if (MODE == 0) {
        e = thin ? e_thin : 0.0;
        a = thin ? a_thin : rc;
        b = thin ? b_thin : 1.0 - rc;
        return;
    }
    const double ee = exp_neg10(fmin(dtau, 50.0));
    const double a_mid = fma(1.0 - ee, rc, -ee), b_mid = (1.0 - a_mid) - ee;
    const double e_mid = dtau > 50.0 ? 0.0 : ee;
    if (MODE == 1) {
        e = e_mid; a = a_mid; b = b_mid;
    } else {
        e = thin ? e_thin : e_mid;
        a = thin ? a_thin : a_mid;
        b = thin ? b_thin : b_mid;
    }
}

template <int MODE>
__device__ __forceinline__ void entry_terms(double dt1, double dt2, double w1, double w2, double wg1, double wg2,
                                            double S_c, double S_1, double S_2, double I_1, double I_2, double &c,
                                            double &g1, double &g2)
{
    double ca1, cb1, ce1, ca2, cb2, ce2;
    lin_weights_fma<MODE>(dt1, ca1, cb1, ce1);
    lin_weights_fma<MODE>(dt2, ca2, cb2, ce2);
    const double t1 = fma(cb1, S_c, fma(ce1, I_1, ca1 * S_1)) * w1;
    const double t2 = fma(cb2, S_c, fma(ce2, I_2, ca2 * S_2)) * w2;
    c = t1 + t2;
// ... 3 lines not shown

__device__ __forceinline__ void entry_lambda(double rh1, double rh2, double w1, double w2, double wg1, double wg2,
                                             double a_c, double a_1, double a_2, double S_c, double S_1, double S_2,
                                             double I_1, double I_2, double &c, double &g1, double &g2)
{
    const double d1 = rh1 * (a_c + a_1), d2 = rh2 * (a_c + a_2);
    const bool mid = ((d1 >= 5e-4) & (d1 <= 50.0)) | ((d2 >= 5e-4) & (d2 <= 50.0));
    const bool thin = (d1 < 5e-4) | (d2 < 5e-4);
    if (__ballot(mid) == 0ull) entry_terms<0>(d1, d2, w1, w2, wg1, wg2, S_c, S_1, S_2, I_1, I_2, c, g1, g2);
    else if (__ballot(thin) == 0ull) entry_terms<1>(d1, d2, w1, w2, wg1, wg2, S_c, S_1, S_2, I_1, I_2, c, g1, g2);
    else entry_terms<2>(d1, d2, w1, w2, wg1, wg2, S_c, S_1, S_2, I_1, I_2, c, g1, g2);
}

template <int MODE>
__device__ __forceinline__ void entry_terms_seq(double dt1, double dt2, const double *pw1, const double *pw2, bool in1,
                                                bool in2, double S_c, double S_1, double S_2, double I_1, double I_2,
                                                double &c, double &g1, double &g2, double &next)
{
    double ca, cb, ce;
    lin_weights_fma<MODE>(dt1, ca, cb, ce);
    const double w1 = *pw1;
    double t1 = fma(cb, S_c, fma(ce, I_1, ca * S_1)) * w1;
    g1 = in1 ? ce * w1 : 0.0;
    asm volatile("" : "+v"(t1), "+v"(g1), "+v"(dt2));
    lin_weights_fma<MODE>(dt2, ca, cb, ce);
    const double w2 = *pw2;
    const double t2 = fma(cb, S_c, fma(ce, I_2, ca * S_2)) * w2;
    c = t1 + t2;
    g2 = in2 ? ce * w2 : 0.0;
    asm volatile("" : "+v"(c), "+v"(g2), "+v"(next));
}
__device__ __forceinline__ void entry_lambda_seq(double d1, double d2, const double *pw1, const double *pw2, bool in1,
                                                 bool in2, double S_c, double S_1, double S_2, double I_1, double I_2,
                                                 double &c, double &g1, double &g2, double &next)
{
    const bool mid = ((d1 >= 5e-4) & (d1 <= 50.0)) | ((d2 >= 5e-4) & (d2 <= 50.0));
    const bool thin = (d1 < 5e-4) | (d2 < 5e-4);
    if (__ballot(mid) == 0ull) entry_terms_seq<0>(d1, d2, pw1, pw2, in1, in2, S_c, S_1, S_2, I_1, I_2, c, g1, g2, next);
    else if (__ballot(thin) == 0ull) entry_terms_seq<1>(d1, d2, pw1, pw2, in1, in2, S_c, S_1, S_2, I_1, I_2, c, g1, g2, next);
    else entry_terms_seq<2>(d1, d2, pw1, pw2, in1, in2, S_c, S_1, S_2, I_1, I_2, c, g1, g2, next);
}

struct LateTerms { double ce1, p1, cb1, ce2, p2, cb2; };
template <int MODE>
__device__ __forceinline__ void late_coeffs(double dt1, double dt2, double S_1, double S_2, LateTerms &L, double &next)
{
    double ca, cb, ce;
    lin_weights_fma<MODE>(dt1, ca, cb, ce);
    L.ce1 = ce; L.p1 = ca * S_1; L.cb1 = cb;
    asm volatile("" : "+v"(L.ce1), "+v"(L.p1), "+v"(L.cb1), "+v"(dt2));
    lin_weights_fma<MODE>(dt2, ca, cb, ce);
    L.ce2 = ce; L.p2 = ca * S_2; L.cb2 = cb;
    asm volatile("" : "+v"(L.ce2), "+v"(L.p2), "+v"(L.cb2), "+v"(next));
}
__device__ __forceinline__ void late_lambda(double d1, double d2, double S_1, double S_2, LateTerms &L, double &next)
{
    const bool mid = ((d1 >= 5e-4) & (d1 <= 50.0)) | ((d2 >= 5e-4) & (d2 <= 50.0));
    const bool thin = (d1 < 5e-4) | (d2 < 5e-4);
    if (__ballot(mid) == 0ull) late_coeffs<0>(d1, d2, S_1, S_2, L, next);
    else if (__ballot(thin) == 0ull) late_coeffs<1>(d1, d2, S_1, S_2, L, next);
    else late_coeffs<2>(d1, d2, S_1, S_2, L, next);
}
__device__ __forceinline__ void late_apply(const LateTerms &L, const double *pw1, const double *pw2, bool in1, bool in2,
                                           double S_c, double I_1, double I_2, double &c, double &g1, double &g2)
{
    const double w1 = *pw1, w2 = *pw2;
    const double t1 = fma(L.cb1, S_c, fma(L.ce1, I_1, L.p1)) * w1;
    const double t2 = fma(L.cb2, S_c, fma(L.ce2, I_2, L.p2)) * w2;
    c = t1 + t2;
    g1 = in1 ? L.ce1 * w1 : 0.0;
    g2 = in2 ? L.ce2 * w2 : 0.0;
}

template <typename T2>
__device__ __forceinline__ double2 ldpair(const T2 *base, int idx, int sh)
{
    const unsigned off = (unsigned)idx << sh;
    return to_d2(*reinterpret_cast<const T2 *>(reinterpret_cast<const char *>(base) + off));
}
template <typename T2> struct Log2Size;
template <> struct Log2Size<double2> { static constexpr int value = 4; };
template <> struct Log2Size<float2> { static constexpr int value = 3; };

__host__ __device__ __forceinline__ void split_blocks(const PatchArgs &pa, int split, int nblock, int &b0, int &b1)
{
    const int nstep = (nblock + pa.Q - 1) / pa.Q;
    const int base = nstep / pa.nsplit, rem = nstep - base * pa.nsplit;
    const int s0 = split * base + (split < rem ? split : rem), s1 = s0 + base + (split < rem ? 1 : 0);
    b0 = s0 * pa.Q;
    b1 = nblock < s1 * pa.Q ? nblock : s1 * pa.Q;
}

#ifndef VRT_REDUCE_LAST
#define VRT_REDUCE_LAST 1
#endif
__device__ __forceinline__ int reduce_block_index(const PatchArgs &pa)
{
    return VRT_REDUCE_LAST ? (int)blockIdx.x - ((int)gridDim.x - pa.red.nred) : ((int)blockIdx.x < pa.red.nred ? (int)blockIdx.x : -1);
}
__device__ __forceinline__ int patch_block_index(const PatchArgs &pa)
{
    return VRT_REDUCE_LAST ? (int)blockIdx.x : (int)blockIdx.x - pa.red.nred;
}
template <typename T, int NT>
__device__ __forceinline__ void patch_reduce_role(const PatchArgs &pa)
{
    typedef typename Pair<T>::type T2;
    const TileArgs &ta = pa.ta;
    const int tid = threadIdx.x;
    int b = reduce_block_index(pa), r = 0;
    if (b >= pa.red.nblk[0]) { b -= pa.red.nblk[0]; r = 1; }
    if (b >= pa.red.nblk[r]) return;
    if (diag(pa.dbg, kDiagNoReduce)) return;
    const int len = pa.red.hi[r] - pa.red.lo[r];
    const int per = NT * pa.red.ppb;
    const int nblock = pair_block_count(pa.npair, pa.lgB);
    int k0 = 0, lw = 0;
    for (int k = 0; k < nblock; k++) {
        pair_block_of(k, pa.npair, pa.lgB, k0, lw);
        const int cnt = (int)((((int64_t)len << lw) + per - 1) / per);
        if (b < cnt) break;
        b -= cnt;
    }
    const int64_t nn = ta.n;
    const size_t run = (size_t)len << lw;
    const size_t base = (size_t)k0 * (size_t)nn + ((size_t)pa.red.lo[r] << lw);
    T2 *Jd = reinterpret_cast<T2 *>(pa.red.Jd[r]);
    const T2 *I0 = reinterpret_cast<const T2 *>(ta.I);
    const size_t plane = (size_t)pa.npair * (size_t)nn;
    if (pa.red.ppb == 4) {
        const size_t f0 = (size_t)b * 4 * NT + tid;
        const unsigned left = f0 < run ? (unsigned)min((size_t)(run - f0 + NT - 1) / NT, (size_t)4) : 0u;
        const size_t e0 = base + (left ? f0 : 0);
        double ax[4], ay[4];
#pragma unroll
        for (int i = 0; i < 4; i++) { ax[i] = 0.0; ay[i] = 0.0; }
        for (int j = 0; j < pa.red.count[r]; j++) {
            const int a = pa.red.angles[r][j];
            const T2 *Ia = I0 + (size_t)a * plane + e0;
            double2 v[4];
#pragma unroll
            for (int i = 0; i < 4; i++) v[i] = to_d2(Ia[(unsigned)i < left ? i * NT : 0]);
#pragma unroll
            for (int i = 0; i < 4; i++) {
                ax[i] += pa.red.w[a] * v[i].x;
                ay[i] += pa.red.w[a] * v[i].y;
            }
        }
#pragma unroll
        for (int i = 0; i < 4; i++)
            if ((unsigned)i < left) Jd[e0 + (size_t)i * NT] = from_d2<T>(make_double2(ax[i], ay[i]));
        return;
    }
    for (int i = 0; i < pa.red.ppb; i++) {
        const size_t f = ((size_t)b * pa.red.ppb + i) * NT + tid;
        if (f >= run) break;
        const size_t e = base + f;
        double ax = 0.0, ay = 0.0;
        for (int j = 0; j < pa.red.count[r]; j++) {
            const int a = pa.red.angles[r][j];
            const double2 v = to_d2(I0[(size_t)a * plane + e]);
            ax += pa.red.w[a] * v.x;
            ay += pa.red.w[a] * v.y;
        }
        Jd[e] = from_d2<T>(make_double2(ax, ay));
    }
}

#ifdef VRT_PATCH_WPE
#define VRT_WPE_ATTR __attribute__((amdgpu_waves_per_eu(VRT_PATCH_WPE, VRT_PATCH_WPE)))
#else
#define VRT_WPE_ATTR
#endif
template <typename T, int AM, int K, int Q, int NT>
__global__ void __launch_bounds__(NT) VRT_WPE_ATTR
k_patch_solve(PatchArgs pa)
{
    typedef typename Pair<T>::type T2;
    extern __shared__ __attribute__((aligned(16))) double2 ptile[];
    const TileArgs &ta = pa.ta;
    const int tid = threadIdx.x;
    if (reduce_block_index(pa) >= 0) {
        patch_reduce_role<T, NT>(pa);
        return;
    }
    const int bid = patch_block_index(pa);
    const int x = bid & 7, rr = bid >> 3;
    const int grp = rr % pa.ngrp, sj = rr / pa.ngrp;
    const int4 rec = pa.wrec[2 * (sj * 8 + x)], rec2 = pa.wrec[2 * (sj * 8 + x) + 1];
    if (rec.y <= 0) return;
    const int sib = grp & ((1 << pa.lgB) - 1);
    const int nblock = pair_block_count(pa.npair, pa.lgB);
    int b0, b1;
    split_blocks(pa, grp >> pa.lgB, nblock, b0, b1);
    if (b0 >= b1) return;
    {
        int k0, lw;
        pair_block_of(b0, pa.npair, pa.lgB, k0, lw);
        if (sib >= (1 << lw)) return;
    }
    const int ent_off = rec.x, n_ent = rec.y, own_lo = rec.z, own_cnt = rec.w;
    const int dbg = kDiag ? pa.dbg : 0;
    const int nlev = diag(dbg, kDiagNoLevels) ? 0 : rec2.x, a = rec2.y & 0xFFFF;
    const int d = rec2.y >> 16;
    const int lo = rec2.z, hi = rec2.w;
    const int64_t n = ta.n;
    const int stride = pa.stride;

    double *s_w1 = reinterpret_cast<double *>(ptile + Q * stride);
    double *s_w2 = s_w1 + pa.cap, *s_r1 = s_w2 + pa.cap, *s_r2 = s_r1 + pa.cap;
    int *s_pos = reinterpret_cast<int *>(s_r2 + pa.cap);
    int *s_u1 = s_pos + pa.cap, *s_u2 = s_u1 + pa.cap;
    uint32_t *s_vis = reinterpret_cast<uint32_t *>(s_u2 + pa.cap), *s_loc = s_vis + pa.cap;
#pragma unroll
    for (int k = 0; k < K; k++) {
        const int i = tid + k * NT;
        const bool ok = i < n_ent;
        const int e = ent_off + (ok ? i : n_ent - 1);
        s_pos[i] = pa.e_pos[e];
        s_u1[i] = pa.e_u1[e];
        s_u2[i] = pa.e_u2[e];
        s_vis[i] = ok ? pa.e_vis[e] : 0u;
        const uint32_t lc = pa.e_loc[e], l1 = lc & 0xFFFFu, l2 = lc >> 16;
        s_loc[i] = (l1 == 0xFFFFu ? (uint32_t)n_ent : l1) | ((l2 == 0xFFFFu ? (uint32_t)n_ent : l2) << 16);
        s_w1[i] = pa.e_w1[e]; s_w2[i] = pa.e_w2[e]; s_r1[i] = pa.e_r1[e]; s_r2[i] = pa.e_r2[e];
    }
    if (tid == 0) {
#pragma unroll
        for (int qi = 0; qi < Q; qi++) ptile[qi * stride + n_ent] = make_double2(0.0, 0.0);
    }
    exp2_table_fill();
    __syncthreads();
    constexpr int lgT2 = Log2Size<T2>::value;
    for (int bk = b0; bk < b1; bk += Q) {
        size_t qbase[Q];
        int qsh[Q];
        bool qok[Q];
#pragma unroll
        for (int qi = 0; qi < Q; qi++) {
            int k0, lw;
            pair_block_of(min(bk + qi, b1 - 1), pa.npair, pa.lgB, k0, lw);
            qok[qi] = bk + qi < b1 && sib < (1 << lw);
            if (!qok[qi] && qi > 0) { qbase[qi] = qbase[qi - 1]; qsh[qi] = qsh[qi - 1]; continue; }
            qbase[qi] = (size_t)k0 * (size_t)n + (size_t)sib;
            qsh[qi] = lw + lgT2;
        }
        if (!qok[0]) break;
        double2 c[K][Q], g1[K][Q], g2[K][Q];
#pragma unroll
        for (int k = 0; k < K; k++) {
            const int i = tid + k * NT;
            const int p = s_pos[i];
            int v1 = s_u1[i], v2 = s_u2[i];
            if (diag(dbg, kDiagCentreGathers)) { v1 = p; v2 = p; }
            int i1 = v1 < lo ? v1 : (int)n - 1, i2 = v2 < lo ? v2 : (int)n - 1;
            if (diag(dbg, kDiagNoGatherI)) { i1 = (int)n - 1; i2 = (int)n - 1; }
            const int av1 = diag(dbg, kDiagNoGatherAlpha) ? p : v1, av2 = diag(dbg, kDiagNoGatherAlpha) ? p : v2;
            const int sv1 = diag(dbg, kDiagNoGatherS) ? p : v1, sv2 = diag(dbg, kDiagNoGatherS) ? p : v2;
            const bool in1 = (v1 >= lo) & (v1 < hi), in2 = (v2 >= lo) & (v2 < hi);
#pragma unroll
            for (int qi = 0; qi < Q; qi++) {
                const int sh = qsh[qi];
                const T2 *__restrict__ S = reinterpret_cast<const T2 *>(ta.S[d]) + qbase[qi];
                const T2 *__restrict__ I = reinterpret_cast<const T2 *>(ta.I) + (size_t)a * pa.npair * (size_t)n + qbase[qi];
                double2 a_c, a_1, a_2;
                if constexpr (AM == VRT_ALPHA_SITE) {
                    const T *__restrict__ Al = reinterpret_cast<const T *>(ta.alpha[d]);
                    const double c0 = Al[p], c1 = Al[av1], c2 = Al[av2];
                    (void)sh;
                    a_c = make_double2(c0, c0); a_1 = make_double2(c1, c1); a_2 = make_double2(c2, c2);
                } else {
                    const T2 *__restrict__ Al =
                        AM == VRT_ALPHA_SITE_LAM
                            ? reinterpret_cast<const T2 *>(ta.alpha[d]) + qbase[qi]
                            : reinterpret_cast<const T2 *>(ta.alpha_angle) + (size_t)a * pa.npair * (size_t)n + qbase[qi];
                    a_c = ldpair(Al, p, sh); a_1 = ldpair(Al, av1, sh); a_2 = ldpair(Al, av2, sh);
                }
                const double2 S_c = ldpair(S, p, sh), S_1 = ldpair(S, sv1, sh), S_2 = ldpair(S, sv2, sh);
                const double2 I_1 = ldpair(I, i1, sh), I_2 = ldpair(I, i2, sh);
                const double w1 = s_w1[i], w2 = s_w2[i], r1 = s_r1[i], r2 = s_r2[i];
                const double wg1 = in1 ? w1 : 0.0, wg2 = in2 ? w2 : 0.0;
                const double rh1 = 0.5 * r1, rh2 = 0.5 * r2;
                if (diag(dbg, kDiagNoWeights)) {
                    c[k][qi] = make_double2(a_c.x + S_c.x + I_1.x + a_1.x + S_1.x, a_c.y + S_c.y + I_2.y + a_2.y + S_2.y);
                    g1[k][qi] = make_double2(w1, w2); g2[k][qi] = make_double2(r1, r2);
                    continue;
                }
                entry_lambda(rh1, rh2, w1, w2, wg1, wg2, a_c.x, a_1.x, a_2.x, S_c.x, S_1.x, S_2.x, I_1.x, I_2.x,
                             c[k][qi].x, g1[k][qi].x, g2[k][qi].x);
                entry_lambda(rh1, rh2, w1, w2, wg1, wg2, a_c.y, a_1.y, a_2.y, S_c.y, S_1.y, S_2.y, I_1.y, I_2.y,
                             c[k][qi].y, g1[k][qi].y, g2[k][qi].y);
            }
        }
        uint32_t vis[K], loc[K];
#pragma unroll
        for (int k = 0; k < K; k++) {
            vis[k] = s_vis[tid + k * NT];
            loc[k] = s_loc[tid + k * NT];
            if (tid + k * NT < n_ent) {
#pragma unroll
                for (int qi = 0; qi < Q; qi++) ptile[qi * stride + tid + k * NT] = make_double2(0.0, 0.0);
            }
        }
        __syncthreads();
        for (int t = 1; t <= nlev; t++) {
#pragma unroll
            for (int k = 0; k < K; k++) {
                if ((vis[k] & 0xFFu) == (uint32_t)t) {
                    const uint32_t l1 = loc[k] & 0xFFFFu, l2 = loc[k] >> 16;
#pragma unroll
                    for (int qi = 0; qi < Q; qi++) {
                        const double2 xv = ptile[qi * stride + l1], yv = ptile[qi * stride + l2];
                        double2 r;
                        r.x = fma(g2[k][qi].x, yv.x, fma(g1[k][qi].x, xv.x, c[k][qi].x));
                        r.y = fma(g2[k][qi].y, yv.y, fma(g1[k][qi].y, xv.y, c[k][qi].y));
                        ptile[qi * stride + tid + k * NT] = r;
                    }
                    vis[k] >>= 8;
                }
            }
            __syncthreads();
        }
#pragma unroll
        for (int k = 0; k < K; k++) {
            const int i = tid + k * NT;
            if (i < own_cnt) {
#pragma unroll
                for (int qi = 0; qi < Q; qi++) {
                    if (qok[qi] && !(diag(dbg, kDiagNoStores) && ptile[qi * stride + i].x != 1.2345e300)) {
                        T2 *I = reinterpret_cast<T2 *>(ta.I) + (size_t)a * pa.npair * (size_t)n + qbase[qi];
                        const unsigned off = (unsigned)(own_lo + i) << qsh[qi];
                        *reinterpret_cast<T2 *>(reinterpret_cast<char *>(I) + off) = from_d2<T>(ptile[qi * stride + i]);
                    }
                }
            }
        }
    }
}


struct PatchItem {
    int sib, b0, b1;
    int ent_off, n_ent, own_lo, own_cnt, nlev, a, d, lo, hi;
};
__device__ __forceinline__ bool patch_item(const PatchArgs &pa, int lgS, PatchItem &it)
{
    const int bid = patch_block_index(pa);
    const int x = bid & 7, rr = bid >> 3;
    const int grp = rr % pa.ngrp, sj = rr / pa.ngrp;
    const int4 rec = pa.wrec[2 * (sj * 8 + x)], rec2 = pa.wrec[2 * (sj * 8 + x) + 1];
    if (rec.y <= 0) return false;
    it.sib = grp & ((1 << lgS) - 1);
    split_blocks(pa, grp >> lgS, pair_block_count(pa.npair, pa.lgB), it.b0, it.b1);
    if (it.b0 >= it.b1) return false;
    it.ent_off = rec.x; it.n_ent = rec.y; it.own_lo = rec.z; it.own_cnt = rec.w;
    it.nlev = rec2.x; it.a = rec2.y & 0xFFFF;
    it.d = rec2.y >> 16;
    it.lo = rec2.z;
    it.hi = rec2.w;
    return true;
}
template <int CAP>
struct EntryTable {
    double *w1, *w2, *r1, *r2;
    int *pos, *u1, *u2;
    uint32_t *vis, *loc;
    __device__ __forceinline__ EntryTable(double2 *tiles, int planes)
    {
        w1 = reinterpret_cast<double *>(tiles + planes * (CAP + 1));
        w2 = w1 + CAP; r1 = w2 + CAP; r2 = r1 + CAP;
        pos = reinterpret_cast<int *>(r2 + CAP);
        u1 = pos + CAP; u2 = u1 + CAP;
        vis = reinterpret_cast<uint32_t *>(u2 + CAP);
        loc = vis + CAP;
    }
    template <typename Tables>
    __device__ __forceinline__ void park(const Tables &pa, const PatchItem &it, int tid) const
    {
        const bool ok = tid < it.n_ent;
        const int e = it.ent_off + (ok ? tid : it.n_ent - 1);
        pos[tid] = pa.e_pos[e];
        u1[tid] = pa.e_u1[e];
        u2[tid] = pa.e_u2[e];
        vis[tid] = ok ? pa.e_vis[e] : 0u;
        const uint32_t lc = pa.e_loc[e], l1 = lc & 0xFFFFu, l2 = lc >> 16;
        loc[tid] = (l1 == 0xFFFFu ? (uint32_t)it.n_ent : l1) | ((l2 == 0xFFFFu ? (uint32_t)it.n_ent : l2) << 16);
        w1[tid] = pa.e_w1[e]; w2[tid] = pa.e_w2[e]; r1[tid] = pa.e_r1[e]; r2[tid] = pa.e_r2[e];
    }
};

struct PairIO {
    int n;
    int npair, lgB, dbg;
    const void *S;
    const void *alpha;
    void *I;
};
template <int AM>
__device__ __forceinline__ PairIO pair_io(const PatchArgs &pa, int d)
{
    PairIO io;
    io.n = (int)pa.ta.n; io.npair = pa.npair; io.lgB = pa.lgB; io.dbg = kDiag ? pa.dbg : 0;
    io.S = pa.ta.S[d];
    io.alpha = AM == VRT_ALPHA_ANGLE_SITE_LAM ? (const void *)pa.ta.alpha_angle : (const void *)pa.ta.alpha[d];
    io.I = pa.ta.I;
    return io;
}

typedef unsigned int vrt_u32x2 __attribute__((ext_vector_type(2)));
typedef unsigned int vrt_u32x4 __attribute__((ext_vector_type(4)));
#ifndef VRT_CHAIN_AUX
#define VRT_CHAIN_AUX 17
#endif
constexpr int kAuxSc1 = VRT_CHAIN_AUX;
constexpr int kChainDepLds = 128;
constexpr int kChainHeadStride = 32;
constexpr int kChainAbortWord = 8 * kChainHeadStride;

struct ChainDev;
constexpr int kCtlItem = 0, kCtlSelf = 1, kCtlNdep = 2, kCtlDepOff = 3, kCtlArgsLo = 4, kCtlArgsHi = 5, kCtlProgLo = 6, kCtlProgHi = 7,
              kCtlBase = 8, kCtlGaveUp = 9, kCtlWords = 12;
template <int CAP>
__device__ __forceinline__ uint32_t *chain_ctl_slots(const EntryTable<CAP> &tab) { return tab.loc + CAP; }
template <int CAP>
__device__ __forceinline__ int32_t *chain_dep_slots(const EntryTable<CAP> &tab) { return reinterpret_cast<int32_t *>(tab.loc + CAP + kCtlWords); }

__device__ __forceinline__ uint32_t ld_agent(const uint32_t *p)
{
    return __hip_atomic_load(p, __ATOMIC_RELAXED, __HIP_MEMORY_SCOPE_AGENT);
}
__device__ __forceinline__ void st_agent(uint32_t *p, uint32_t v)
{
    __hip_atomic_store(p, v, __ATOMIC_RELAXED, __HIP_MEMORY_SCOPE_AGENT);
}
__device__ __forceinline__ uint32_t *chain_progress(const uint32_t *ctl)
{
    return reinterpret_cast<uint32_t *>(((uint64_t)ctl[kCtlProgHi] << 32) | (uint64_t)ctl[kCtlProgLo]);
// ... 230 lines not shown
                    if (!diag(dbg, kDiagNoWeights)) {
                        LateTerms Lx, Ly;
                        late_lambda(d1x, d2x, (double)rS_1.x, (double)rS_2.x, Lx, d1y);
                        double sink = 0.0;
                        late_lambda(d1y, d2y, (double)rS_1.y, (double)rS_2.y, Ly, sink);
                        if (!diag(dbg, kDiagNoWait)) chain_data_wait<T2>(rsI, (unsigned)i1 << sh, (unsigned)i2 << sh, rI_1, rI_2, s_dep);
                        late_apply(Lx, tab.w1 + tid, tab.w2 + tid, in1, in2, (double)rS_c.x, (double)rI_1.x, (double)rI_2.x, c.x, g1.x, g2.x);
                        late_apply(Ly, tab.w1 + tid, tab.w2 + tid, in1, in2, (double)rS_c.y, (double)rI_1.y, (double)rI_2.y, c.y, g1.y, g2.y);
                    } else {
                        if (!diag(dbg, kDiagNoWait)) chain_data_wait<T2>(rsI, (unsigned)i1 << sh, (unsigned)i2 << sh, rI_1, rI_2, s_dep);
                        c = make_double2(d1x + (double)rS_c.x + (double)rS_1.x + (double)rI_1.x, d2y + (double)rS_c.y + (double)rS_2.y + (double)rI_2.y);
                        g1 = make_double2(in1 ? d2x : 0.0, in1 ? d1y : 0.0);
                        g2 = make_double2(in2 ? d1x : 0.0, in2 ? d2y : 0.0);
                    }
                }
            } else {
                rI_1 = at(Ia + qb, (unsigned)i1 << sh);
                rI_2 = at(Ia + qb, (unsigned)i2 << sh);
            }
            const bool in1 = (v1 >= it.lo) & (v1 < it.hi), in2 = (v2 >= it.lo) & (v2 < it.hi);
            if constexpr (CHAIN == 2) {
            } else if (diag(dbg, kDiagNoWeights)) {
                c = make_double2(d1x + (double)rS_c.x + (double)rS_1.x + (double)rI_1.x, d2y + (double)rS_c.y + (double)rS_2.y + (double)rI_2.y);
                g1 = make_double2(in1 ? d2x : 0.0, in1 ? d1y : 0.0);
                g2 = make_double2(in2 ? d1x : 0.0, in2 ? d2y : 0.0);
            } else {
                entry_lambda_seq(d1x, d2x, tab.w1 + tid, tab.w2 + tid, in1, in2, (double)rS_c.x, (double)rS_1.x, (double)rS_2.x,
                                 (double)rI_1.x, (double)rI_2.x, c.x, g1.x, g2.x, d1y);
                double sink = 0.0;
                entry_lambda_seq(d1y, d2y, tab.w1 + tid, tab.w2 + tid, in1, in2, (double)rS_c.y, (double)rS_1.y, (double)rS_2.y,
                                 (double)rI_1.y, (double)rI_2.y, c.y, g1.y, g2.y, sink);
            }
        }
        uint32_t vis = tab.vis[tid];
        const uint32_t loc = tab.loc[tid];
        {
            double z;
            asm volatile("v_mov_b64 %0, 0" : "=v"(z));
            if (tid < it.n_ent) ptile[tid] = make_double2(z, z);
        }
        if constexpr (CHAIN == 1) asm volatile("s_waitcnt vmcnt(0)" ::: "memory");
        __syncthreads();
        if constexpr (CHAIN == 1) {
            if (bk > it.b0 && tid == 0) chain_publish(s_dep, bk - it.b0);
        }
        const int nlev = diag(dbg, kDiagNoLevels) ? 0 : it.nlev;
        __builtin_amdgcn_s_setprio(VRT_LEVEL_PRIO);
        for (int t = 1; t <= nlev; t++) {
            if ((vis & 0xFFu) == (uint32_t)t) {
                const double2 xv = ptile[loc & 0xFFFFu], yv = ptile[loc >> 16];
                double2 r;
                r.x = fma(g2.x, yv.x, fma(g1.x, xv.x, c.x));
                r.y = fma(g2.y, yv.y, fma(g1.y, xv.y, c.y));
                ptile[tid] = r;
                vis >>= 8;
            }
            __syncthreads();
        }
        __builtin_amdgcn_s_setprio(0);
        if (tid < it.own_cnt && !(diag(dbg, kDiagNoStores) && ptile[tid].x != 1.2345e300)) {
            if (CHAIN && !diag(dbg, kDiagPlainStoreI)) {
                const __amdgpu_buffer_rsrc_t rsI = plane_rsrc(Ia + qb, n << sh);
                BufSc1<T2>::store(rsI, (unsigned)(it.own_lo + tid) << sh, from_d2<T>(ptile[tid]));
            } else {
                T2 *I = reinterpret_cast<T2 *>(pa.I) + (size_t)it.a * pa.npair * (size_t)n + qb;
                *reinterpret_cast<T2 *>(reinterpret_cast<char *>(I) + ((unsigned)(it.own_lo + tid) << sh)) = from_d2<T>(ptile[tid]);
            }
        }
        __syncthreads();
    }
}

template <typename T, int AM, int NT>
__global__ void __launch_bounds__(NT) VRT_LEAN_ATTR
k_patch_lean(PatchArgs pa)
{
    extern __shared__ __attribute__((aligned(16))) double2 ptile[];
    const int tid = threadIdx.x;
    if (reduce_block_index(pa) >= 0) {
        patch_reduce_role<T, NT>(pa);
        return;
    }
    PatchItem it;
    if (!patch_item(pa, pa.lgB, it)) return;
    if (diag(pa.dbg, kDiagNoPairLoop)) it.b1 = it.b0;
    const EntryTable<NT> tab(ptile, 1);
    tab.park(pa, it, tid);
    if (tid == 0) ptile[it.n_ent] = make_double2(0.0, 0.0);
    exp2_table_fill();
    __syncthreads();
    lean_pairs<T, AM, NT, 0>(pair_io<AM>(pa, it.d), it, tab, ptile);
}


template <int AM, int NT, bool CHAIN>
__device__ __forceinline__ void quad_pairs(const PairIO &pa, const PatchItem &it, const EntryTable<NT> &tab,
                                           double2 *ptile)
{
    const int tid = threadIdx.x;
    const int sib2 = it.sib, b0 = it.b0, b1 = it.b1;
    const unsigned n = (unsigned)pa.n;
    const int n_ent = it.n_ent, own_lo = it.own_lo, own_cnt = it.own_cnt, nlev = it.nlev, a = it.a;
    const int lo = it.lo, hi = it.hi;
    constexpr int CAP = NT;
    double2 *tileA = ptile, *tileB = ptile + (CAP + 1);
    double *const s_r1 = tab.r1, *const s_r2 = tab.r2, *const s_w1 = tab.w1, *const s_w2 = tab.w2;
    int *const s_pos = tab.pos, *const s_u1 = tab.u1, *const s_u2 = tab.u2;
    uint32_t *const s_vis = tab.vis, *const s_loc = tab.loc;
    const float2 *Sd = reinterpret_cast<const float2 *>(pa.S);
    const float2 *Ia = reinterpret_cast<const float2 *>(pa.I) + (size_t)a * pa.npair * (size_t)n;
    auto at4 = [](const float2 *base, unsigned off) { return *reinterpret_cast<const float4 *>(reinterpret_cast<const char *>(base) + off); };
    const int32_t *s_dep = chain_dep_slots(tab);
    for (int bk = b0; bk < b1; bk++) {
        int k0, lw;
        if constexpr (CHAIN) { k0 = 2 * bk; lw = 1; }
        else {
            pair_block_of(bk, pa.npair, pa.lgB, k0, lw);
            if (2 * sib2 >= (1 << lw)) break;
        }
        const size_t qb = (size_t)k0 * (size_t)n + (size_t)(CHAIN ? 0 : 2 * sib2);
        const int sh = lw + 3;
        uint32_t seen = 0;
        if constexpr (CHAIN) seen = chain_peek(s_dep, bk - b0 + 1);
        const int p = s_pos[tid], v1 = s_u1[tid], v2 = s_u2[tid];
        double d1x, d2x, d1y, d2y, d1z, d2z, d1w, d2w;
        {
            float4 a_c, a_1, a_2;
            if constexpr (AM == VRT_ALPHA_SITE) {
                const float *__restrict__ A1 = reinterpret_cast<const float *>(pa.alpha);
                const float c0 = A1[p], c1 = A1[v1], c2 = A1[v2];
                a_c = make_float4(c0, c0, c0, c0); a_1 = make_float4(c1, c1, c1, c1); a_2 = make_float4(c2, c2, c2, c2);
            } else {
                const float2 *Al = AM == VRT_ALPHA_SITE_LAM ? reinterpret_cast<const float2 *>(pa.alpha) + qb
                                                            : reinterpret_cast<const float2 *>(pa.alpha) + (size_t)a * pa.npair * (size_t)n + qb;
                a_c = at4(Al, (unsigned)p << sh); a_1 = at4(Al, (unsigned)v1 << sh); a_2 = at4(Al, (unsigned)v2 << sh);
            }
            const double rh1 = 0.5 * s_r1[tid], rh2 = 0.5 * s_r2[tid];
            d1x = rh1 * ((double)a_c.x + (double)a_1.x); d2x = rh2 * ((double)a_c.x + (double)a_2.x);
            d1y = rh1 * ((double)a_c.y + (double)a_1.y); d2y = rh2 * ((double)a_c.y + (double)a_2.y);
            d1z = rh1 * ((double)a_c.z + (double)a_1.z); d2z = rh2 * ((double)a_c.z + (double)a_2.z);
            d1w = rh1 * ((double)a_c.w + (double)a_1.w); d2w = rh2 * ((double)a_c.w + (double)a_2.w);
        }
        asm volatile("" : "+v"(d1x), "+v"(d2x), "+v"(d1y), "+v"(d2y), "+v"(d1z), "+v"(d2z), "+v"(d1w), "+v"(d2w) : : "memory");
        double2 cA, g1A, g2A, cB, g1B, g2B;
        {
            const int i1 = v1 < lo ? v1 : (int)n - 1, i2 = v2 < lo ? v2 : (int)n - 1;
            const bool in1 = (v1 >= lo) & (v1 < hi), in2 = (v2 >= lo) & (v2 < hi);
            const float4 S_c = at4(Sd + qb, (unsigned)p << sh), S_1 = at4(Sd + qb, (unsigned)v1 << sh), S_2 = at4(Sd + qb, (unsigned)v2 << sh);
            float4 I_1, I_2;
            if constexpr (CHAIN) {
                chain_wait(s_dep, bk - b0 + 1, seen);
                const __amdgpu_buffer_rsrc_t rsI = plane_rsrc(Ia + qb, n << sh);
                I_1 = BufSc1<float4>::load(rsI, (unsigned)i1 << sh);
                I_2 = BufSc1<float4>::load(rsI, (unsigned)i2 << sh);
            } else {
                I_1 = at4(Ia + qb, (unsigned)i1 << sh);
                I_2 = at4(Ia + qb, (unsigned)i2 << sh);
            }
            entry_lambda_seq(d1x, d2x, s_w1 + tid, s_w2 + tid, in1, in2, (double)S_c.x, (double)S_1.x, (double)S_2.x,
                             (double)I_1.x, (double)I_2.x, cA.x, g1A.x, g2A.x, d1y);
            entry_lambda_seq(d1y, d2y, s_w1 + tid, s_w2 + tid, in1, in2, (double)S_c.y, (double)S_1.y, (double)S_2.y,
                             (double)I_1.y, (double)I_2.y, cA.y, g1A.y, g2A.y, d1z);
            entry_lambda_seq(d1z, d2z, s_w1 + tid, s_w2 + tid, in1, in2, (double)S_c.z, (double)S_1.z, (double)S_2.z,
                             (double)I_1.z, (double)I_2.z, cB.x, g1B.x, g2B.x, d1w);
            double sink = 0.0;
            entry_lambda_seq(d1w, d2w, s_w1 + tid, s_w2 + tid, in1, in2, (double)S_c.w, (double)S_1.w, (double)S_2.w,
                             (double)I_1.w, (double)I_2.w, cB.y, g1B.y, g2B.y, sink);
        }
        uint32_t vis = s_vis[tid];
        const uint32_t loc = s_loc[tid];
        {
            double z;
            asm volatile("v_mov_b64 %0, 0" : "=v"(z));
            if (tid < n_ent) {
                tileA[tid] = make_double2(z, z);
                tileB[tid] = make_double2(z, z);
            }
        }
        if constexpr (CHAIN) asm volatile("s_waitcnt vmcnt(0)" ::: "memory");
        __syncthreads();
        if constexpr (CHAIN) {
            if (bk > b0 && tid == 0) chain_publish(s_dep, bk - b0);
        }
        for (int t = 1; t <= nlev; t++) {
            if ((vis & 0xFFu) == (uint32_t)t) {
                const uint32_t l1 = loc & 0xFFFFu, l2 = loc >> 16;
                const double2 xa = tileA[l1], ya = tileA[l2], xb = tileB[l1], yb = tileB[l2];
                double2 ra, rb;
                ra.x = fma(g2A.x, ya.x, fma(g1A.x, xa.x, cA.x));
                ra.y = fma(g2A.y, ya.y, fma(g1A.y, xa.y, cA.y));
                rb.x = fma(g2B.x, yb.x, fma(g1B.x, xb.x, cB.x));
                rb.y = fma(g2B.y, yb.y, fma(g1B.y, xb.y, cB.y));
                tileA[tid] = ra;
                tileB[tid] = rb;
                vis >>= 8;
            }
            __syncthreads();
        }
        if (tid < own_cnt) {
            const double2 ra = tileA[tid], rb = tileB[tid];
            const float4 out = make_float4((float)ra.x, (float)ra.y, (float)rb.x, (float)rb.y);
            if constexpr (CHAIN) {
                const __amdgpu_buffer_rsrc_t rsI = plane_rsrc(Ia + qb, n << sh);
                BufSc1<float4>::store(rsI, (unsigned)(own_lo + tid) << sh, out);
            } else {
                float2 *I = reinterpret_cast<float2 *>(pa.I) + (size_t)a * pa.npair * (size_t)n + qb;
                *reinterpret_cast<float4 *>(reinterpret_cast<char *>(I) + ((unsigned)(own_lo + tid) << sh)) = out;
            }
        }
        __syncthreads();
    }
}

#ifndef VRT_QUAD_ATTR
#define VRT_QUAD_ATTR __attribute__((amdgpu_waves_per_eu(6, 6)))
#endif
template <int AM, int NT>
__global__ void __launch_bounds__(NT) VRT_QUAD_ATTR
k_patch_quad(PatchArgs pa)
{
    extern __shared__ __attribute__((aligned(16))) double2 ptile[];
    const int tid = threadIdx.x;
    if (reduce_block_index(pa) >= 0) {
        patch_reduce_role<float, NT>(pa);
        return;
    }
    PatchItem it;
    if (!patch_item(pa, pa.lgB - 1, it)) return;
    const EntryTable<NT> tab(ptile, 2);
    tab.park(pa, it, tid);
    if (tid == 0) {
        ptile[it.n_ent] = make_double2(0.0, 0.0);
        ptile[NT + 1 + it.n_ent] = make_double2(0.0, 0.0);
    }
    exp2_table_fill();
    __syncthreads();
    quad_pairs<AM, NT, false>(pair_io<AM>(pa, it.d), it, tab, ptile);
}


struct ChainDev {
    TileArgs ta;
    int npair, nsplit, cap;
    const int32_t *e_pos, *e_u1, *e_u2;
    const uint32_t *e_vis, *e_loc;
    const double *e_w1, *e_w2, *e_r1, *e_r2;
    PatchReduce red;
    const int4 *items;
    int q_off[9];
    const int32_t *deps;
    uint32_t *progress;
    uint32_t *ctrl;
    uint32_t *host_status;
    int64_t n_patches;
    uint32_t spin_limit;
    int static_items;
    int dbg;
};

__device__ __forceinline__ const uint32_t *chain_abort_word(const uint32_t *cd_words)
{
    return reinterpret_cast<const ChainDev *>(cd_words)->ctrl + kChainAbortWord;
}

__device__ __forceinline__ int cd_int(const int *p) { return __builtin_amdgcn_readfirstlane(*p); }
template <typename P>
__device__ __forceinline__ P *cd_ptr(P *const *p) { return uniform_ptr(*p); }

__device__ __forceinline__ void chain_wait_slow(const int32_t *s_dep, int step)
{
    const int lane = (int)(threadIdx.x & 63u);
    const uint32_t *ctl = reinterpret_cast<const uint32_t *>(s_dep - kCtlWords);
    const ChainDev *cd = reinterpret_cast<const ChainDev *>(((uint64_t)ctl[kCtlArgsHi] << 32) | (uint64_t)ctl[kCtlArgsLo]);
    uint32_t *abort_word = cd->ctrl + kChainAbortWord;
    const uint32_t *progress = chain_progress(ctl);
    const uint32_t target = ctl[kCtlBase] + (uint32_t)step, limit = cd->spin_limit;
    const int ndep = (int)ctl[kCtlNdep];
    for (int c0 = 0; c0 < ndep; c0 += 64) {
        const int j = c0 + lane;
        const int dep = j < 64 + kChainDepLds ? s_dep[j] : (j < ndep ? (cd->deps + ctl[kCtlDepOff])[j] : (int)ctl[kCtlSelf]);
        const uint32_t *w = progress + dep;
        uint32_t spins = 0;
        for (;;) {
            const uint32_t v = ld_agent(w);
            if (__all(j >= ndep || (int)(v - target) >= 0)) break;
            __builtin_amdgcn_s_sleep(8);
            if ((++spins & 127u) == 1u) {
                if (spins > limit) {
                    st_agent(abort_word, 1u);
                    uint32_t *hs = cd->host_status;
                    __hip_atomic_store(hs + 1, ctl[kCtlItem], __ATOMIC_RELAXED, __HIP_MEMORY_SCOPE_SYSTEM);
                    __hip_atomic_store(hs, 1u, __ATOMIC_RELAXED, __HIP_MEMORY_SCOPE_SYSTEM);
                }
                if (ld_agent(abort_word) != 0u) return;
            }
        }
    }
}

__device__ __forceinline__ void chain_data_give_up_cd(const ChainDev *cd, uint32_t item)
{
    st_agent(cd->ctrl + kChainAbortWord, 1u);
    uint32_t *hs = cd->host_status;
    __hip_atomic_store(hs + 1, item, __ATOMIC_RELAXED, __HIP_MEMORY_SCOPE_SYSTEM);
    __hip_atomic_store(hs, 1u, __ATOMIC_RELAXED, __HIP_MEMORY_SCOPE_SYSTEM);
}

template <typename T, int NT, int LGB, int MODE>
__device__ __forceinline__ void chain_reduce(const ChainDev &cd, const ChainDev *cdp, uint32_t item, int r, int lo, int hi, int b0, int b1)
{
    typedef typename Pair<T>::type T2;
// ... 136 lines not shown
        __syncthreads();
        if (tid == 0 && s_ctl[kCtlGaveUp]) chain_data_give_up_cd(cd, (uint32_t)idx);
    }
    if constexpr (MODE == 1) {
        asm volatile("s_waitcnt vmcnt(0)" ::: "memory");
        __syncthreads();
        if (tid == 0) chain_publish(s_dep, b1 - b0);
    }
}

template <typename T, int AM, int NT>
__global__ void __launch_bounds__(NT) VRT_LEAN_ATTR
k_patch_chain(ChainDev ca, const ChainDev *cd, uint32_t base)
{
    extern __shared__ __attribute__((aligned(16))) double2 ptile[];
    chain_item<T, AM, NT, false, 1>(ca, cd, base, ptile);
}
template <typename T, int AM, int NT>
__global__ void __launch_bounds__(NT) __attribute__((amdgpu_waves_per_eu(6, 6)))
k_patch_chain_df(ChainDev ca, const ChainDev *cd, uint32_t base)
{
    extern __shared__ __attribute__((aligned(16))) double2 ptile[];
    chain_item<T, AM, NT, false, 2>(ca, cd, base, ptile);
}
template <int AM, int NT>
__global__ void __launch_bounds__(NT) VRT_QUAD_ATTR
k_patch_chain_quad(ChainDev ca, const ChainDev *cd, uint32_t base)
{
    extern __shared__ __attribute__((aligned(16))) double2 ptile[];
    chain_item<float, AM, NT, true, 1>(ca, cd, base, ptile);
}

#define VRT_PATCH_SHAPES(X) \
    X(1, 1, 256) X(1, 1, 512) X(1, 1, 1024) X(2, 1, 256) X(2, 1, 512) X(1, 2, 256) X(1, 2, 512) X(1, 2, 1024) X(2, 2, 512)

template <typename T, int AM>
static int launch_shape(int K, int Q, int NT, dim3 grid, size_t lds, hipStream_t st, const PatchArgs &pa)
{
    if constexpr (sizeof(T) == 4) {
        if (pa.quad) {
            switch (NT) {
            case 256: hipLaunchKernelGGL((k_patch_quad<AM, 256>), grid, dim3(256), lds, st, pa); return VRT_OK;
            case 512: hipLaunchKernelGGL((k_patch_quad<AM, 512>), grid, dim3(512), lds, st, pa); return VRT_OK;
            case 1024: hipLaunchKernelGGL((k_patch_quad<AM, 1024>), grid, dim3(1024), lds, st, pa); return VRT_OK;
            default: break;
            }
        }
    }
    if (pa.lean && K == 1 && Q == 1) {
        switch (NT) {
        case 256: hipLaunchKernelGGL((k_patch_lean<T, AM, 256>), grid, dim3(256), lds, st, pa); return VRT_OK;
        case 512: hipLaunchKernelGGL((k_patch_lean<T, AM, 512>), grid, dim3(512), lds, st, pa); return VRT_OK;
        case 1024: hipLaunchKernelGGL((k_patch_lean<T, AM, 1024>), grid, dim3(1024), lds, st, pa); return VRT_OK;
        default: break;
        }
    }
#define VRT_PATCH_CASE(k, q, nt) \
    if (K == k && Q == q && NT == nt) { hipLaunchKernelGGL((k_patch_solve<T, AM, k, q, nt>), grid, dim3(nt), lds, st, pa); return VRT_OK; }
    VRT_PATCH_SHAPES(VRT_PATCH_CASE)
#undef VRT_PATCH_CASE
    return fail(VRT_EINVAL, "no patch kernel for this (entries per thread, pairs, threads) shape");
}

template <typename T>
static int launch_mode(int am, int K, int Q, int NT, dim3 grid, size_t lds, hipStream_t st, const PatchArgs &pa)
{
    switch (am) {
    case VRT_ALPHA_SITE: return launch_shape<T, VRT_ALPHA_SITE>(K, Q, NT, grid, lds, st, pa);
    case VRT_ALPHA_SITE_LAM: return launch_shape<T, VRT_ALPHA_SITE_LAM>(K, Q, NT, grid, lds, st, pa);
    default: return launch_shape<T, VRT_ALPHA_ANGLE_SITE_LAM>(K, Q, NT, grid, lds, st, pa);
    }
}

bool patch_shape_exists(int K, int Q, int NT)
{
#define VRT_PATCH_CASE(k, q, nt) if (K == k && Q == q && NT == nt) return true;
    VRT_PATCH_SHAPES(VRT_PATCH_CASE)
#undef VRT_PATCH_CASE
    return false;
}

int ensure_patch_work(vrt_plan *p, int G, const std::vector<int32_t> &group_angles, const std::vector<int> &group_off)
{
    if (p->d_patch_work && p->patch_work_groups == G) return VRT_OK;
    if (p->d_patch_work) { (void)hipFree(p->d_patch_work); p->d_patch_work = nullptr; }
    const int maxL = p->tile_max_layers;
    std::vector<int4> work;
    p->patch_work_off.assign((size_t)G * (size_t)(maxL + 2) + 1, 0);
    std::vector<std::pair<int64_t, int32_t>> items;
    for (int gi = 0; gi < G; gi++)
        for (int layer = 0; layer <= maxL + 1; layer++) {
            p->patch_work_off[(size_t)gi * (size_t)(maxL + 2) + (size_t)layer] = (int64_t)(work.size() / 2);
            if (layer < 2 || layer > maxL) continue;
            items.clear();
            for (int j = group_off[(size_t)gi]; j < group_off[(size_t)gi + 1]; j++) {
                const int a = group_angles[(size_t)j];
                const int32_t *first = p->h_patch_first.data() + (size_t)a * (size_t)(maxL + 2);
                for (int32_t q = first[layer]; q < first[layer + 1]; q++)
                    items.push_back({(int64_t)p->h_patch_rec[(size_t)q].z * 64 + (j - group_off[(size_t)gi]), q});
            }
            std::sort(items.begin(), items.end());
            const size_t m = items.size();
            if (m == 0) continue;
            const size_t slots = (m + 7) / 8;
            const size_t base = work.size();
            work.resize(base + slots * 8 * 2, make_int4(0, 0, 0, 0));
            for (int x = 0; x < 8; x++) {
                const size_t b0 = m * (size_t)x / 8, b1 = m * (size_t)(x + 1) / 8;
                for (size_t t = b0; t < b1; t++) {
                    const int32_t q = items[t].second;
                    const int2 r2 = p->h_patch_rec2[(size_t)q];
                    const int d = p->dir_of_active[(size_t)r2.y] > 0 ? 0 : 1;
                    const Direction &dir = d == 0 ? p->g->up : p->g->down;
                    const size_t slot = base + 2 * ((t - b0) * 8 + (size_t)x);
                    work[slot] = p->h_patch_rec[(size_t)q];
                    work[slot + 1] = make_int4(r2.x, r2.y | (d << 16), (int)(dir.reduced[(size_t)layer - 1] - 1), (int)(dir.reduced[(size_t)layer] - 1));
                }
            }
        }
    p->patch_work_off.back() = (int64_t)(work.size() / 2);
    if (int rc = dev_alloc(&p->d_patch_work, work.size())) return rc;
    VRT_HIP_TRY(hipMemcpy(p->d_patch_work, work.data(), sizeof(int4) * work.size(), hipMemcpyHostToDevice));
    p->patch_work_groups = G;
    return VRT_OK;
}

static void size_reduce(PatchReduce &red, int npair, int lgB, int NT)
{
    red.nred = 0;
    int64_t total = 0;
    for (int r = 0; r < 2; r++)
        if (red.count[r] > 0 && red.Jd[r]) total += (int64_t)std::max(0, red.hi[r] - red.lo[r]) * npair;
    red.ppb = total <= (int64_t)NT * 1024 ? 1 : 4;
    const int64_t per = (int64_t)NT * red.ppb;
    const int nblock = pair_block_count(npair, lgB);
    for (int r = 0; r < 2; r++) {
        const int64_t len = red.hi[r] - red.lo[r];
        red.nblk[r] = 0;
        if (len > 0 && red.count[r] > 0 && red.Jd[r])
            for (int k = 0; k < nblock; k++) {
                int k0, lw;
                pair_block_of(k, npair, lgB, k0, lw);
                red.nblk[r] += (int)(((len << lw) + per - 1) / per);
            }
        red.nred += red.nblk[r];
    }
    red.nred = (red.nred + 7) / 8 * 8;
}

int launch_patch_layer(vrt_plan *p, const TileArgs &ta, int npair, int layer, int group, int Q, hipStream_t st,
                       bool f32, const PatchReduce *reduce)
{
    const int target_wgs = p->tune.patch_target;
    const int maxL = p->tile_max_layers;
    const size_t wo = (size_t)group * (size_t)(maxL + 2) + (size_t)layer;
    const int64_t w0 = (layer >= 2 && layer <= maxL) ? p->patch_work_off[wo] : 0, w1 = (layer >= 2 && layer <= maxL) ? p->patch_work_off[wo + 1] : 0;
    PatchArgs pa;
    if (reduce) {
        pa.red = *reduce;
        size_reduce(pa.red, npair, native_lg(p, f32), p->patch_NT);
    }
    if (w1 <= w0 && pa.red.nred == 0) return VRT_OK;
    pa.ta = ta;
    pa.npair = npair;
    pa.layer = layer;
    pa.lgB = native_lg(p, f32);
    pa.quad = (f32 && pa.lgB >= 1 && p->patch_K == 1 && p->tune.patch_quad != 0 && (npair & 1) == 0) ? 1 : 0;
    if (pa.quad) Q = 1;
    pa.lean = (p->tune.patch_lean != 0 && p->patch_K == 1 && Q == 1 && !pa.quad && npair >= 2) ? 1 : 0;
    const int lgS = pa.lgB - pa.quad;
    pa.Q = Q;
    pa.nsplit = 1;
    pa.ngrp = 1 << lgS;
    if (w1 > w0) {
        const int64_t items = (w1 - w0) << lgS;
        const int nblock = pair_block_count(npair, pa.lgB);
        const int steps_all = (nblock + Q - 1) / Q;
        int nsplit;
        if (p->tune.patch_split > 0) nsplit = std::min(steps_all, p->tune.patch_split);
        else if (target_wgs > 0) nsplit = (int)std::max<int64_t>(1, std::min<int64_t>(steps_all, (target_wgs + items - 1) / items));
        else {
            const double T = std::min(900.0, 460.0 + 4100.0 / (double)steps_all);
            const int s_min = (int)std::min<int64_t>(steps_all, std::max<int64_t>(1, (512 + items - 1) / items));
            double dmin = 1e300;
            for (int c = steps_all; c >= 1; c--) {
                const int sc = (steps_all + c - 1) / c;
                if (sc >= s_min) dmin = std::min(dmin, std::fabs(std::log((double)items * sc / T)));
            }
            nsplit = s_min;
            for (int c = steps_all; c >= 1; c--) {
                const int sc = (steps_all + c - 1) / c;
                if (sc >= s_min && std::fabs(std::log((double)items * sc / T)) <= dmin + 0.03) nsplit = sc;
            }
        }
        pa.nsplit = nsplit;
        pa.ngrp = nsplit << lgS;
    }
    pa.stride = p->patch_cap + 1;
    pa.cap = p->patch_cap;
    pa.dbg = kDiag ? p->tune.debug_flags : 0;
    pa.wrec = p->d_patch_work + 2 * w0;
    pa.e_pos = p->e_pos; pa.e_u1 = p->e_u1; pa.e_u2 = p->e_u2;
    pa.e_vis = p->e_vis; pa.e_loc = p->e_loc;
    pa.e_w1 = p->e_w1; pa.e_w2 = p->e_w2; pa.e_r1 = p->e_r1; pa.e_r2 = p->e_r2;
    const dim3 grid((unsigned)(pa.red.nred + (w1 - w0) * pa.ngrp));
    const size_t lds = (size_t)(pa.quad ? 2 : Q) * (size_t)pa.stride * sizeof(double2) + (size_t)pa.cap * (4 * sizeof(double) + 5 * sizeof(int32_t));
    const int rc = f32 ? launch_mode<float>(ta.alpha_mode, p->patch_K, Q, p->patch_NT, grid, lds, st, pa)
                       : launch_mode<double>(ta.alpha_mode, p->patch_K, Q, p->patch_NT, grid, lds, st, pa);
    return rc;
}

bool patch_chain_possible(const vrt_plan *p, int npair, bool f32)
{
    if (!p->patch_ok || p->tune.patch_chain == 0 || p->patch_K != 1 || p->patch_NT != 512) return false;
    const int lgB = native_lg(p, f32);
    const bool quad = f32 && lgB >= 1 && p->tune.patch_quad != 0 && (npair & 1) == 0;
    if (lgB - (quad ? 1 : 0) != 0) return false;
    if (!f32 && p->tune.patch_lean == 0) return false;
    if (p->tile_max_layers >= 65535 || p->A > 63) return false;
    if (p->tune.patch_chain == 1) return true;
    if (f32) return false;
    const double per_layer = (double)p->n_patches / (double)std::max(1, p->tile_max_layers);
    return per_layer * (double)pair_block_count(npair, lgB) <= 1400.0;
}

bool patch_chain_dataflag(const vrt_plan *p, int npair, bool f32)
{
    if (f32 || p->tune.chain_dataflag == 0 || native_lg(p, f32) != 0) return false;
    return p->tune.chain_dataflag == 1 || npair <= 2;
}

static int chain_nsplit(const vrt_plan *p, int nblock)
{
    const int per = std::max(1, p->tune.chain_pairs);
    const double per_layer = (double)p->n_patches / (double)std::max(1, p->tile_max_layers);
    const int fill = (int)std::ceil(1024.0 / std::max(1.0, per_layer));
    return std::max(1, std::min({std::max((nblock + per - 1) / per, fill), nblock, 511}));
}

static int ensure_patch_chain(vrt_plan *p, int npair, int lgB, int nsplit, bool with_reduce)
{
    if (p->d_chain_items && p->chain_npair == npair && p->chain_lgB == lgB && p->chain_nsplit == nsplit &&
        p->chain_reduce == (with_reduce ? 1 : 0))
        return VRT_OK;
    {
        auto stash = [&]() {
            if (!p->d_chain_items) return;
            vrt_plan::ChainSet cs;
            cs.npair = p->chain_npair; cs.lgB = p->chain_lgB; cs.nsplit = p->chain_nsplit; cs.reduce = p->chain_reduce;
            cs.items = p->d_chain_items; cs.deps = p->d_chain_deps; cs.n_items = p->chain_items;
            for (int x = 0; x <= 8; x++) cs.q_off[x] = p->chain_q_off[x];
            p->d_chain_items = nullptr; p->d_chain_deps = nullptr;
            p->chain_npair = -1;
            p->chain_cache.push_back(cs);
            if (p->chain_cache.size() > 3) {
                (void)hipFree(p->chain_cache.front().items);
                (void)hipFree(p->chain_cache.front().deps);
                p->chain_cache.erase(p->chain_cache.begin());
            }
        };
        for (size_t c = 0; c < p->chain_cache.size(); c++) {
            const vrt_plan::ChainSet cs = p->chain_cache[c];
            if (cs.npair == npair && cs.lgB == lgB && cs.nsplit == nsplit && cs.reduce == (with_reduce ? 1 : 0)) {
                p->chain_cache.erase(p->chain_cache.begin() + (long)c);
                stash();
                p->d_chain_items = cs.items; p->d_chain_deps = cs.deps; p->chain_items = cs.n_items;
                for (int x = 0; x <= 8; x++) p->chain_q_off[x] = cs.q_off[x];
                p->chain_npair = npair; p->chain_lgB = lgB; p->chain_nsplit = nsplit; p->chain_reduce = with_reduce ? 1 : 0;
                const size_t words = (size_t)nsplit * (size_t)std::max<int64_t>(p->n_patches, 1);
                if (words <= p->chain_progress_cap) return VRT_OK;
                break;
            }
        }
        stash();
    }
    const vrt_grid *g = p->g;
    const int maxL = p->tile_max_layers, A = p->A;
    const int64_t n = g->n, n_patches = p->n_patches;
    const int nblock = pair_block_count(npair, lgB);
    if ((int64_t)nsplit * n_patches >= ((int64_t)1 << 31)) return fail(VRT_EINVAL, "too many (split, patch) progress words");
    PatchArgs sp;
    sp.nsplit = nsplit;
    sp.Q = 1;
    std::vector<int> steps((size_t)nsplit);
    for (int s = 0; s < nsplit; s++) {
        int b0, b1;
        split_blocks(sp, s, nblock, b0, b1);
        steps[(size_t)s] = b1 - b0;
    }
    std::vector<int4> q[8];
    std::vector<int32_t> rdeps;
    const size_t dep_base = p->h_patch_deps.size();
    std::vector<std::pair<int64_t, int32_t>> items;
    std::vector<int> dir_angles[2];
    for (int a = 0; a < A; a++) dir_angles[p->dir_of_active[(size_t)a] > 0 ? 0 : 1].push_back(a);
    std::vector<int32_t> run_start((size_t)(maxL + 2) * 2 * 8, 0);
    auto first_of = [&](int a, int layer) { return p->h_patch_first[(size_t)a * (size_t)(maxL + 2) + (size_t)layer]; };
    auto level_queues = [&]() {
        size_t longest = 0;
        for (int x = 0; x < 8; x++) longest = std::max(longest, q[x].size());
        for (int x = 0; x < 8; x++)
            while (q[x].size() < longest) {
                q[x].push_back(make_int4(0, 0, 0x40000000, 0));
                q[x].push_back(make_int4(0, 0, 0, 0));
                q[x].push_back(make_int4(0, 0, 0, 0));
            }
    };
    auto emit_reduce = [&](int layer) {
        if (!with_reduce) return;
        for (int d = 0; d < 2; d++) {
            const Direction &dir = d == 0 ? g->up : g->down;
            const int Ld = (int)dir.reduced.size() - 1;
            if (dir_angles[d].empty() || layer < 1 || layer > Ld) continue;
            const int64_t lo = dir.reduced[(size_t)layer - 1] - 1;
            const int64_t hi = layer == Ld ? n : dir.reduced[(size_t)layer] - 1;
            const int32_t *rs = run_start.data() + ((size_t)layer * 2 + (size_t)d) * 8;
            constexpr int64_t R = 512;
            for (int64_t clo = lo; clo < hi; clo += R) {
                const int64_t chi = std::min(hi, clo + R);
                int x = 0;
                if (layer >= 2) { while (x < 7 && rs[x + 1] <= clo) x++; }
                else x = (int)std::min<int64_t>(7, 8 * (clo - lo) / std::max<int64_t>(1, hi - lo));
                const size_t d0 = rdeps.size();
                if (layer >= 2)
                    for (int a : dir_angles[d])
                        for (int32_t pq = first_of(a, layer); pq < first_of(a, layer + 1); pq++) {
                            const int4 &rec = p->h_patch_rec[(size_t)pq];
                            if (rec.z < chi && rec.z + rec.w > clo) rdeps.push_back(pq);
                        }
                for (int s = 0; s < nsplit; s++) {
                    q[x].push_back(make_int4((int)clo, (int)chi, (int)0x80000000u, (d << 6) | (s << 7)));
                    q[x].push_back(make_int4((int)(dep_base + d0), (int)(rdeps.size() - d0), 0, steps[(size_t)s]));
                    q[x].push_back(make_int4(0, 0, 0, 0));
                }
            }
        }
    };
    for (int layer = 2; layer <= maxL; layer++) {
        for (int d = 0; d < 2; d++) {
            const Direction &dir = d == 0 ? g->up : g->down;
            if (layer > (int)dir.reduced.size() - 1) continue;
            items.clear();
            for (size_t j = 0; j < dir_angles[d].size(); j++) {
                const int a = dir_angles[d][j];
                for (int32_t pq = first_of(a, layer); pq < first_of(a, layer + 1); pq++)
                    items.push_back({(int64_t)p->h_patch_rec[(size_t)pq].z * 64 + (int64_t)j, pq});
            }
            std::sort(items.begin(), items.end());
            const size_t m = items.size();
            int32_t *rs = run_start.data() + ((size_t)layer * 2 + (size_t)d) * 8;
            for (int x = 0; x < 8; x++) {
                const size_t t0 = m * (size_t)x / 8, t1 = m * (size_t)(x + 1) / 8;
                rs[x] = t0 < m ? p->h_patch_rec[(size_t)items[t0].second].z : INT32_MAX;
                for (size_t t = t0; t < t1; t++) {
                    const int32_t pq = items[t].second;
                    const int4 &rec = p->h_patch_rec[(size_t)pq];
                    const int2 &rec2 = p->h_patch_rec2[(size_t)pq];
                    const int64_t o0 = p->h_patch_dep_off[(size_t)pq], o1 = p->h_patch_dep_off[(size_t)pq + 1];
                    for (int s = 0; s < nsplit; s++) {
                        q[x].push_back(make_int4(rec.x, rec.z, rec.y | (rec.w << 10) | (rec2.x << 20),
                                                 rec2.y | (d << 6) | (s << 7) | (layer << 16)));
                        q[x].push_back(make_int4((int)o0, (int)(o1 - o0), pq, 0));
                        q[x].push_back(make_int4((int)(dir.reduced[(size_t)layer - 1] - 1), (int)(dir.reduced[(size_t)layer] - 1), 0, 0));
                    }
                }
            }
            level_queues();
        }
        emit_reduce(layer - 1);
        level_queues();
// ... 158 lines not shown
```

Before: 88.00 billion.

## Balance patch work splits by per-patch level cost with precomputed work lists

Replaces the uniform per-layer split of pair blocks across workgroups with a host-built, cached per-workgroup record list. Each record carries its own block range and sibling. A greedy heap allocator gives costlier patches (cost modeled from level count) more splits within a workgroup budget, and shares are ordered longest-first. The aim is to cut tail imbalance in each layer launch. In exchange it adds host-side list construction, a third int4 record per workgroup, and a cache of up to eight list sets.

```diff
diff --git a/include/voronoirt.h b/include/voronoirt.h
--- a/include/voronoirt.h
+++ b/include/voronoirt.h
@@ -131,6 +131,8 @@
 int vrt_patch_schedule_get_deps(const vrt_patch_schedule *s, int64_t *dep_off, int32_t *dep_list);
 int vrt_patch_schedule_get_layers(const vrt_patch_schedule *s, uint32_t *vis, int32_t *nlev, int64_t *n_visits);
 void vrt_patch_schedule_destroy(vrt_patch_schedule *s);
+int vrt_patch_split_query(int n_items, int steps, const double *cost, int64_t budget, int longest_first,
+                          int32_t *shares, int64_t capacity, int64_t *count);
 
 int vrt_delaunay_up(vrt_grid *g, const double k[3], const double *S, const double *I0,
                     int64_t nI0, const double *alpha, int n_sweeps, double *I_out);
diff --git a/voronoirt_amd/_lib.py b/voronoirt_amd/_lib.py
--- a/voronoirt_amd/_lib.py
+++ b/voronoirt_amd/_lib.py
@@ -126,6 +126,7 @@
     "vrt_patch_schedule_get_deps": (ctypes.c_int, [vp, p_i64, p_i32]),
     "vrt_patch_schedule_get_layers": (ctypes.c_int, [vp, ctypes.POINTER(ctypes.c_uint32), p_i32, p_i64]),
     "vrt_patch_schedule_destroy": (None, [vp]),
+    "vrt_patch_split_query": (ctypes.c_int, [ctypes.c_int, ctypes.c_int, p_dbl, c_i64, ctypes.c_int, p_i32, c_i64, p_i64]),
     "vrt_lambda_update_dev": (ctypes.c_int, [vp, c_i64, c_i64, vp, vp, vp, vp, vp, p_dbl, vp]),
     "vrt_short_characteristics": (ctypes.c_int, [c_i64, c_i64, c_i64, p_dbl, p_dbl, p_dbl, c_i64, p_dbl,
                                                  p_int, p_dbl, c_i64, p_dbl, c_i64, p_dbl, ctypes.c_int,
diff --git a/voronoirt_amd/csrc/vrt_api.cpp b/voronoirt_amd/csrc/vrt_api.cpp
--- a/voronoirt_amd/csrc/vrt_api.cpp
+++ b/voronoirt_amd/csrc/vrt_api.cpp
@@ -27,7 +27,7 @@
     static const char *names[] = {"VRT_PATH", "VRT_STEP_K", "VRT_STEP_SINGLE", "VRT_STEP_PAIRS", "VRT_STEP_XCD",
                                   "VRT_STEP_STREAMS", "VRT_STEP_LEVEL_MAP", "VRT_STEP_GROUP_DIR", "VRT_TILE_WIDE",
                                   "VRT_TILE_PRE", "VRT_PATCH_K", "VRT_PATCH_NT", "VRT_PATCH_OWN",
-                                  "VRT_PATCH_Q", "VRT_PATCH_TARGET", "VRT_PATCH_SPLIT", "VRT_PAIR_BLOCK", "VRT_PATCH_QUAD", "VRT_PATCH_LEAN", "VRT_PATCH_CHAIN", "VRT_CHAIN_PAIRS", "VRT_CHAIN_SPIN", "VRT_CHAIN_DATAFLAG", "VRT_CHAIN_STATIC", "VRT_LAMBDA_NATIVE", "VRT_DEBUG_FLAGS", "VRT_DEBUG_SKIP_LEVELS",
+                                  "VRT_PATCH_Q", "VRT_PATCH_TARGET", "VRT_PATCH_SPLIT", "VRT_PATCH_COST", "VRT_PAIR_BLOCK", "VRT_PATCH_QUAD", "VRT_PATCH_LEAN", "VRT_PATCH_CHAIN", "VRT_CHAIN_PAIRS", "VRT_CHAIN_SPIN", "VRT_CHAIN_DATAFLAG", "VRT_CHAIN_STATIC", "VRT_LAMBDA_NATIVE", "VRT_DEBUG_FLAGS", "VRT_DEBUG_SKIP_LEVELS",
                                   "VRT_TILE_DEBUG"};
     for (const char *nm : names) {
         const char *e = std::getenv(nm);
@@ -65,7 +65,7 @@
         {"VRT_TILE_PRE", &t.tile_pre, 0, 1, false},
         {"VRT_PATCH_K", &t.patch_K, 1, 8, true}, {"VRT_PATCH_NT", &t.patch_NT, 64, 1024, true},
         {"VRT_PATCH_OWN", &t.patch_own, 0, 65535, true}, {"VRT_PATCH_Q", &t.patch_Q, 1, 4, false},
-        {"VRT_PATCH_TARGET", &t.patch_target, 0, 1 << 20, false}, {"VRT_PATCH_SPLIT", &t.patch_split, 0, 4096, false}, {"VRT_PAIR_BLOCK", &t.pair_block, 1, 16, true},
+        {"VRT_PATCH_TARGET", &t.patch_target, 0, 1 << 20, false}, {"VRT_PATCH_SPLIT", &t.patch_split, 0, 4096, false}, {"VRT_PATCH_COST", &t.patch_cost, 0, 1, false}, {"VRT_PAIR_BLOCK", &t.pair_block, 1, 16, true},
         {"VRT_PATCH_QUAD", &t.patch_quad, 0, 1, true}, {"VRT_PATCH_LEAN", &t.patch_lean, 0, 1, false},
         {"VRT_PATCH_CHAIN", &t.patch_chain, 0, 2, false}, {"VRT_CHAIN_PAIRS", &t.chain_pairs, 1, 256, false},
         {"VRT_CHAIN_SPIN", &t.chain_spin, 1, 1 << 20, false}, {"VRT_CHAIN_DATAFLAG", &t.chain_dataflag, 0, 2, false},
@@ -241,7 +241,7 @@
     for (int i = 0; i < 2; i++) dev_free(p->ws_cg[i]);
     dev_free(p->d_step_angles);
     dev_free(p->d_level_map);
-    dev_free(p->d_patch_work);
+    drop_patch_work(p);
     dev_free(p->d_chain_items); dev_free(p->d_chain_deps); dev_free(p->d_chain_progress); dev_free(p->d_chain_ctrl);
     for (auto &cs : p->chain_cache) { dev_free(cs.items); dev_free(cs.deps); }
     p->chain_cache.clear();
@@ -1181,6 +1181,27 @@
 
 void vrt_patch_schedule_destroy(vrt_patch_schedule *s) { delete s; }
 
+int vrt_patch_split_query(int n_items, int steps, const double *cost, int64_t budget, int longest_first,
+                          int32_t *shares, int64_t capacity, int64_t *count)
+{
+    if (!cost || !shares || !count) return fail(VRT_EINVAL, "NULL argument");
+    if (n_items < 1 || steps < 1 || capacity < 0) return fail(VRT_EINVAL, "need n_items >= 1, steps >= 1 and capacity >= 0");
+    for (int i = 0; i < n_items; i++)
+        if (!(cost[i] > 0.0) || !std::isfinite(cost[i])) return fail(VRT_EINVAL, "item costs must be positive and finite");
+    return guarded([&] {
+        std::vector<int> s;
+        std::vector<PatchShare> out;
+        choose_patch_split(n_items, steps, cost, budget, s);
+        deal_patch_shares(n_items, steps, cost, s, longest_first != 0, out);
+        *count = (int64_t)out.size();
+        if ((int64_t)out.size() > capacity) return fail(VRT_EINVAL, "more workgroups than `capacity`");
+        for (size_t j = 0; j < out.size(); j++) {
+            shares[3 * j] = out[j].item; shares[3 * j + 1] = out[j].s0; shares[3 * j + 2] = out[j].s1;
+        }
+        return (int)VRT_OK;
+    });
+}
+
 int vrt_grid_get_storage_order(const vrt_grid *g, int dir, int64_t *out)
 {
     if (!g || !out) return fail(VRT_EINVAL, "NULL argument");
diff --git a/voronoirt_amd/csrc/vrt_internal.h b/voronoirt_amd/csrc/vrt_internal.h
--- a/voronoirt_amd/csrc/vrt_internal.h
+++ b/voronoirt_amd/csrc/vrt_internal.h
@@ -171,6 +171,7 @@
     int chain_dataflag = 2;
     int patch_split = 0;
     int patch_target = 0;
+    int patch_cost = 1;
     int chain_static = 1;
     int lambda_native = 1;
     int debug_flags = 0, debug_skip_levels = 0, tile_debug = 0;
@@ -353,9 +354,15 @@
     };
     std::vector<ChainSet> chain_cache;
     uint32_t chain_epoch = 0;
-    int4 *d_patch_work = nullptr;
+    std::vector<int32_t> patch_work;
     std::vector<int64_t> patch_work_off;
     int patch_work_groups = 0;
+    struct PatchListSet {
+        int npair = -1, lgB = -1, lgS = -1, Q = -1, split = -1, target = -1, cost = -1;
+        int4 *recs = nullptr;
+        std::vector<int64_t> off;
+    };
+    std::vector<PatchListSet> patch_lists;
     hipStream_t step_stream[4] = {nullptr, nullptr, nullptr, nullptr};
     hipEvent_t step_fork = nullptr, step_join[4] = {nullptr, nullptr, nullptr, nullptr};
     int last_path = 0;
@@ -503,6 +510,11 @@
 bool patch_shape_exists(int K, int Q, int NT);
 int launch_patch_entries(vrt_plan *p, int a, int64_t first, int64_t count);
 int ensure_patch_work(vrt_plan *p, int G, const std::vector<int32_t> &group_angles, const std::vector<int> &group_off);
+void drop_patch_work(vrt_plan *p);
+struct PatchShare { int32_t item, s0, s1; };
+void choose_patch_split(int n_items, int steps, const double *cost, int64_t budget, std::vector<int> &s);
+void deal_patch_shares(int n_items, int steps, const double *cost, const std::vector<int> &s, bool longest_first,
+                       std::vector<PatchShare> &out);
 int launch_patch_layer(vrt_plan *p, const TileArgs &ta, int npair, int layer, int group, int Q, hipStream_t st,
                        bool f32, const PatchReduce *reduce);
 bool patch_chain_possible(const vrt_plan *p, int npair, bool f32);
diff --git a/voronoirt_amd/csrc/vrt_layers.hip b/voronoirt_amd/csrc/vrt_layers.hip
--- a/voronoirt_amd/csrc/vrt_layers.hip
+++ b/voronoirt_amd/csrc/vrt_layers.hip
@@ -192,7 +192,7 @@
     if (!p->d_step_angles && (rc = dev_alloc(&p->d_step_angles, (size_t)A))) return rc;
     VRT_HIP_TRY(hipMemcpy(p->d_step_angles, list.data(), sizeof(int32_t) * list.size(), hipMemcpyHostToDevice));
     p->h_step_angles = list;
-    dev_free(p->d_patch_work);
+    drop_patch_work(p);
     if (!p->step_fork) VRT_HIP_TRY(hipEventCreateWithFlags(&p->step_fork, hipEventDisableTiming));
     for (int gi = 0; gi < 4; gi++) {
         if (gi >= 1 && gi < G && !p->step_stream[gi]) {
diff --git a/voronoirt_amd/csrc/vrt_patch.hip b/voronoirt_amd/csrc/vrt_patch.hip
--- a/voronoirt_amd/csrc/vrt_patch.hip
+++ b/voronoirt_amd/csrc/vrt_patch.hip
@@ -22,8 +22,7 @@
     TileArgs ta;
     int npair;
     int layer;
-    int ngrp;
-    int nsplit, Q;
+    int Q;
     int lgB;
     int stride;
     int cap;
@@ -193,13 +192,11 @@
 template <> struct Log2Size<double2> { static constexpr int value = 4; };
 template <> struct Log2Size<float2> { static constexpr int value = 3; };
 
-__host__ __device__ __forceinline__ void split_blocks(const PatchArgs &pa, int split, int nblock, int &b0, int &b1)
-{
-    const int nstep = (nblock + pa.Q - 1) / pa.Q;
-    const int base = nstep / pa.nsplit, rem = nstep - base * pa.nsplit;
-    const int s0 = split * base + (split < rem ? split : rem), s1 = s0 + base + (split < rem ? 1 : 0);
-    b0 = s0 * pa.Q;
-    b1 = nblock < s1 * pa.Q ? nblock : s1 * pa.Q;
+static inline void split_steps(int nstep, int nsplit, int split, int &s0, int &s1)
+{
+    const int base = nstep / nsplit, rem = nstep - base * nsplit;
+    s0 = split * base + (split < rem ? split : rem);
+    s1 = s0 + base + (split < rem ? 1 : 0);
 }
 
 #ifndef VRT_REDUCE_LAST
@@ -295,21 +292,10 @@
         patch_reduce_role<T, NT>(pa);
         return;
     }
-    const int bid = patch_block_index(pa);
-    const int x = bid & 7, rr = bid >> 3;
-    const int grp = rr % pa.ngrp, sj = rr / pa.ngrp;
-    const int4 rec = pa.wrec[2 * (sj * 8 + x)], rec2 = pa.wrec[2 * (sj * 8 + x) + 1];
+    const int4 *wr = pa.wrec + 3 * (size_t)patch_block_index(pa);
+    const int4 rec = wr[0], rec2 = wr[1], rec3 = wr[2];
     if (rec.y <= 0) return;
-    const int sib = grp & ((1 << pa.lgB) - 1);
-    const int nblock = pair_block_count(pa.npair, pa.lgB);
-    int b0, b1;
-    split_blocks(pa, grp >> pa.lgB, nblock, b0, b1);
-    if (b0 >= b1) return;
-    {
-        int k0, lw;
-        pair_block_of(b0, pa.npair, pa.lgB, k0, lw);
-        if (sib >= (1 << lw)) return;
-    }
+    const int b0 = rec3.x, b1 = rec3.y, sib = rec3.z;
     const int ent_off = rec.x, n_ent = rec.y, own_lo = rec.z, own_cnt = rec.w;
     const int dbg = kDiag ? pa.dbg : 0;
     const int nlev = diag(dbg, kDiagNoLevels) ? 0 : rec2.x, a = rec2.y & 0xFFFF;
@@ -454,16 +440,12 @@
     int sib, b0, b1;
     int ent_off, n_ent, own_lo, own_cnt, nlev, a, d, lo, hi;
 };
-__device__ __forceinline__ bool patch_item(const PatchArgs &pa, int lgS, PatchItem &it)
-{
-    const int bid = patch_block_index(pa);
-    const int x = bid & 7, rr = bid >> 3;
-    const int grp = rr % pa.ngrp, sj = rr / pa.ngrp;
-    const int4 rec = pa.wrec[2 * (sj * 8 + x)], rec2 = pa.wrec[2 * (sj * 8 + x) + 1];
+__device__ __forceinline__ bool patch_item(const PatchArgs &pa, PatchItem &it)
+{
+    const int4 *wr = pa.wrec + 3 * (size_t)patch_block_index(pa);
+    const int4 rec = wr[0], rec2 = wr[1], rec3 = wr[2];
     if (rec.y <= 0) return false;
-    it.sib = grp & ((1 << lgS) - 1);
-    split_blocks(pa, grp >> lgS, pair_block_count(pa.npair, pa.lgB), it.b0, it.b1);
-    if (it.b0 >= it.b1) return false;
+    it.b0 = rec3.x; it.b1 = rec3.y; it.sib = rec3.z;
     it.ent_off = rec.x; it.n_ent = rec.y; it.own_lo = rec.z; it.own_cnt = rec.w;
     it.nlev = rec2.x; it.a = rec2.y & 0xFFFF;
     it.d = rec2.y >> 16;
@@ -860,7 +842,7 @@
         return;
     }
     PatchItem it;
-    if (!patch_item(pa, pa.lgB, it)) return;
+    if (!patch_item(pa, it)) return;
     if (diag(pa.dbg, kDiagNoPairLoop)) it.b1 = it.b0;
     const EntryTable<NT> tab(ptile, 1);
     tab.park(pa, it, tid);
@@ -1004,7 +986,7 @@
         return;
     }
     PatchItem it;
-    if (!patch_item(pa, pa.lgB - 1, it)) return;
+    if (!patch_item(pa, it)) return;
     const EntryTable<NT> tab(ptile, 2);
     tab.park(pa, it, tid);
     if (tid == 0) {
@@ -1307,15 +1289,14 @@
 
 int ensure_patch_work(vrt_plan *p, int G, const std::vector<int32_t> &group_angles, const std::vector<int> &group_off)
 {
-    if (p->d_patch_work && p->patch_work_groups == G) return VRT_OK;
-    if (p->d_patch_work) { (void)hipFree(p->d_patch_work); p->d_patch_work = nullptr; }
+    if (!p->patch_work_off.empty() && p->patch_work_groups == G) return VRT_OK;
+    drop_patch_work(p);
     const int maxL = p->tile_max_layers;
-    std::vector<int4> work;
     p->patch_work_off.assign((size_t)G * (size_t)(maxL + 2) + 1, 0);
     std::vector<std::pair<int64_t, int32_t>> items;
     for (int gi = 0; gi < G; gi++)
         for (int layer = 0; layer <= maxL + 1; layer++) {
-            p->patch_work_off[(size_t)gi * (size_t)(maxL + 2) + (size_t)layer] = (int64_t)(work.size() / 2);
+            p->patch_work_off[(size_t)gi * (size_t)(maxL + 2) + (size_t)layer] = (int64_t)p->patch_work.size();
             if (layer < 2 || layer > maxL) continue;
             items.clear();
             for (int j = group_off[(size_t)gi]; j < group_off[(size_t)gi + 1]; j++) {
@@ -1325,28 +1306,181 @@
                     items.push_back({(int64_t)p->h_patch_rec[(size_t)q].z * 64 + (j - group_off[(size_t)gi]), q});
             }
             std::sort(items.begin(), items.end());
-            const size_t m = items.size();
-            if (m == 0) continue;
-            const size_t slots = (m + 7) / 8;
-            const size_t base = work.size();
-            work.resize(base + slots * 8 * 2, make_int4(0, 0, 0, 0));
-            for (int x = 0; x < 8; x++) {
-                const size_t b0 = m * (size_t)x / 8, b1 = m * (size_t)(x + 1) / 8;
-                for (size_t t = b0; t < b1; t++) {
-                    const int32_t q = items[t].second;
-                    const int2 r2 = p->h_patch_rec2[(size_t)q];
-                    const int d = p->dir_of_active[(size_t)r2.y] > 0 ? 0 : 1;
-                    const Direction &dir = d == 0 ? p->g->up : p->g->down;
-                    const size_t slot = base + 2 * ((t - b0) * 8 + (size_t)x);
-                    work[slot] = p->h_patch_rec[(size_t)q];
-                    work[slot + 1] = make_int4(r2.x, r2.y | (d << 16), (int)(dir.reduced[(size_t)layer - 1] - 1), (int)(dir.reduced[(size_t)layer] - 1));
-                }
-            }
-        }
-    p->patch_work_off.back() = (int64_t)(work.size() / 2);
-    if (int rc = dev_alloc(&p->d_patch_work, work.size())) return rc;
-    VRT_HIP_TRY(hipMemcpy(p->d_patch_work, work.data(), sizeof(int4) * work.size(), hipMemcpyHostToDevice));
+            for (const auto &it : items) p->patch_work.push_back(it.second);
+        }
+    p->patch_work_off.back() = (int64_t)p->patch_work.size();
     p->patch_work_groups = G;
+    return VRT_OK;
+}
+
+void drop_patch_work(vrt_plan *p)
+{
+    for (auto &ls : p->patch_lists) dev_free(ls.recs);
+    p->patch_lists.clear();
+    p->patch_work.clear();
+    p->patch_work_off.clear();
+    p->patch_work_groups = 0;
+}
+
+constexpr double kStepCostUs = 2.053, kStepCostPerLevelUs = 0.1474;
+static inline double patch_step_cost(int nlev) { return kStepCostUs + kStepCostPerLevelUs * (double)nlev; }
+
+void choose_patch_split(int n_items, int steps, const double *cost, int64_t budget, std::vector<int> &s)
+{
+    s.assign((size_t)std::max(n_items, 0), 1);
+    if (n_items <= 0 || steps <= 1) return;
+    auto longest = [&](int i) { return (steps + s[(size_t)i] - 1) / s[(size_t)i]; };
+    struct Key { double t; int s, i; };
+    auto below = [](const Key &a, const Key &b) { return a.t != b.t ? a.t < b.t : a.s != b.s ? a.s > b.s : a.i > b.i; };
+    int64_t used = n_items;
+    for (;;) {
+        std::vector<Key> heap;
+        heap.reserve((size_t)n_items);
+        for (int i = 0; i < n_items; i++) heap.push_back({longest(i) * cost[i], s[(size_t)i], i});
+        std::make_heap(heap.begin(), heap.end(), below);
+        while (used < budget && heap.front().s < steps) {
+            std::pop_heap(heap.begin(), heap.end(), below);
+            Key &k = heap.back();
+            s[(size_t)k.i] = ++k.s;
+            k.t = longest(k.i) * cost[k.i];
+            std::push_heap(heap.begin(), heap.end(), below);
+            used++;
+        }
+        const double tmax = heap.front().t;
+        int64_t freed = 0;
+        for (int i = 0; i < n_items; i++) {
+            if (!(longest(i) * cost[i] < tmax)) continue;
+            const int fewest = (steps + longest(i) - 1) / longest(i);
+            freed += s[(size_t)i] - fewest;
+            s[(size_t)i] = fewest;
+        }
+        used -= freed;
+        if (freed == 0 || heap.front().s >= steps) return;
+    }
+}
+
+void deal_patch_shares(int n_items, int steps, const double *cost, const std::vector<int> &s, bool longest_first,
+                       std::vector<PatchShare> &out)
+{
+    out.clear();
+    for (int i = 0; i < n_items; i++)
+        for (int k = 0; k < s[(size_t)i]; k++) {
+            PatchShare sh;
+            sh.item = i;
+            split_steps(steps, s[(size_t)i], k, sh.s0, sh.s1);
+            if (sh.s1 > sh.s0) out.push_back(sh);
+        }
+    if (longest_first)
+        std::stable_sort(out.begin(), out.end(), [&](const PatchShare &a, const PatchShare &b) {
+            return (a.s1 - a.s0) * cost[a.item] > (b.s1 - b.s0) * cost[b.item];
+        });
+}
+
+static int uniform_split(const vrt_plan *p, int64_t items, int steps_all)
+{
+    if (p->tune.patch_split > 0) return std::min(steps_all, p->tune.patch_split);
+    if (p->tune.patch_target > 0)
+        return (int)std::max<int64_t>(1, std::min<int64_t>(steps_all, (p->tune.patch_target + items - 1) / items));
+    const double T = std::min(900.0, 460.0 + 4100.0 / (double)steps_all);
+    const int s_min = (int)std::min<int64_t>(steps_all, std::max<int64_t>(1, (512 + items - 1) / items));
+    double dmin = 1e300;
+    for (int c = steps_all; c >= 1; c--) {
+        const int sc = (steps_all + c - 1) / c;
+        if (sc >= s_min) dmin = std::min(dmin, std::fabs(std::log((double)items * sc / T)));
+    }
+    int nsplit = s_min;
+    for (int c = steps_all; c >= 1; c--) {
+        const int sc = (steps_all + c - 1) / c;
+        if (sc >= s_min && std::fabs(std::log((double)items * sc / T)) <= dmin + 0.03) nsplit = sc;
+    }
+    return nsplit;
+}
+
+static int build_patch_lists(vrt_plan *p, vrt_plan::PatchListSet &ls)
+{
+    const int maxL = p->tile_max_layers;
+    const int nblock = pair_block_count(ls.npair, ls.lgB), steps_all = (nblock + ls.Q - 1) / ls.Q, nsib = 1 << ls.lgS;
+    const bool uniform = ls.split > 0 || ls.target > 0;
+    std::vector<int4> recs;
+    ls.off.assign(p->patch_work_off.size(), 0);
+    std::vector<double> cost;
+    std::vector<int> s;
+    std::vector<PatchShare> shares;
+    std::vector<int4> xl[8];
+    for (size_t wo = 0; wo + 1 < p->patch_work_off.size(); wo++) {
+        ls.off[wo] = (int64_t)(recs.size() / 3);
+        const int64_t w0 = p->patch_work_off[wo], m = p->patch_work_off[wo + 1] - w0;
+        if (m <= 0) continue;
+        const int layer = (int)(wo % (size_t)(maxL + 2));
+        const int64_t slots = (m + 7) / 8;
+        const int nsplit = uniform_split(p, (slots * 8) << ls.lgS, steps_all);
+        size_t longest_list = 0;
+        for (int x = 0; x < 8; x++) {
+            const int64_t t0 = m * x / 8, t1 = m * (x + 1) / 8;
+            const int n_items = (int)(t1 - t0) * nsib;
+            cost.resize((size_t)n_items);
+            for (int i = 0; i < n_items; i++) {
+                const int32_t q = p->patch_work[(size_t)(w0 + t0 + i / nsib)];
+                cost[(size_t)i] = ls.cost ? patch_step_cost(p->h_patch_rec2[(size_t)q].x) : 1.0;
+            }
+            if (uniform) s.assign((size_t)n_items, nsplit);
+            else choose_patch_split(n_items, steps_all, cost.data(), (slots * nsplit) << ls.lgS, s);
+            deal_patch_shares(n_items, steps_all, cost.data(), s, false, shares);
+            if (nsib > 1)
+                std::stable_sort(shares.begin(), shares.end(), [&](const PatchShare &a, const PatchShare &b) {
+                    return a.item / nsib != b.item / nsib ? a.item / nsib < b.item / nsib : a.s0 < b.s0;
+                });
+            if (!uniform)
+                std::stable_sort(shares.begin(), shares.end(), [&](const PatchShare &a, const PatchShare &b) {
+                    return (a.s1 - a.s0) * cost[(size_t)a.item] > (b.s1 - b.s0) * cost[(size_t)b.item];
+                });
+            xl[x].clear();
+            for (const PatchShare &sh : shares) {
+                const int b0 = sh.s0 * ls.Q, b1 = std::min(nblock, sh.s1 * ls.Q), sib = sh.item % nsib;
+                int k0, lw;
+                pair_block_of(b0, ls.npair, ls.lgB, k0, lw);
+                if (b0 >= b1 || sib >= (1 << (lw - (ls.lgB - ls.lgS)))) continue;
+                const int32_t q = p->patch_work[(size_t)(w0 + t0 + sh.item / nsib)];
+                const int2 r2 = p->h_patch_rec2[(size_t)q];
+                const int d = p->dir_of_active[(size_t)r2.y] > 0 ? 0 : 1;
+                const Direction &dir = d == 0 ? p->g->up : p->g->down;
+                xl[x].push_back(p->h_patch_rec[(size_t)q]);
+                xl[x].push_back(make_int4(r2.x, r2.y | (d << 16), (int)(dir.reduced[(size_t)layer - 1] - 1), (int)(dir.reduced[(size_t)layer] - 1)));
+                xl[x].push_back(make_int4(b0, b1, sib, 0));
+            }
+            longest_list = std::max(longest_list, xl[x].size() / 3);
+        }
+        const size_t base = recs.size();
+        recs.resize(base + longest_list * 8 * 3, make_int4(0, 0, 0, 0));
+        for (int x = 0; x < 8; x++)
+            for (size_t r = 0; r < xl[x].size() / 3; r++)
+                for (int k = 0; k < 3; k++) recs[base + 3 * (r * 8 + (size_t)x) + (size_t)k] = xl[x][3 * r + (size_t)k];
+    }
+    ls.off.back() = (int64_t)(recs.size() / 3);
+    if (recs.empty()) return VRT_OK;
+    if (int rc = dev_alloc(&ls.recs, recs.size())) return rc;
+    VRT_HIP_TRY(hipMemcpy(ls.recs, recs.data(), sizeof(int4) * recs.size(), hipMemcpyHostToDevice));
+    return VRT_OK;
+}
+
+static int ensure_patch_lists(vrt_plan *p, int npair, int lgB, int lgS, int Q, const vrt_plan::PatchListSet *&out)
+{
+    for (const auto &ls : p->patch_lists)
+        if (ls.npair == npair && ls.lgB == lgB && ls.lgS == lgS && ls.Q == Q && ls.split == p->tune.patch_split &&
+            ls.target == p->tune.patch_target && ls.cost == p->tune.patch_cost) {
+            out = &ls;
+            return VRT_OK;
+        }
+    if (p->patch_lists.size() >= 8) {
+        dev_free(p->patch_lists.front().recs);
+        p->patch_lists.erase(p->patch_lists.begin());
+    }
+    vrt_plan::PatchListSet ls;
+    ls.npair = npair; ls.lgB = lgB; ls.lgS = lgS; ls.Q = Q;
+    ls.split = p->tune.patch_split; ls.target = p->tune.patch_target; ls.cost = p->tune.patch_cost;
+    if (int rc = build_patch_lists(p, ls)) { dev_free(ls.recs); return rc; }
+    p->patch_lists.push_back(std::move(ls));
+    out = &p->patch_lists.back();
     return VRT_OK;
 }
 
@@ -1376,16 +1510,15 @@
 int launch_patch_layer(vrt_plan *p, const TileArgs &ta, int npair, int layer, int group, int Q, hipStream_t st,
                        bool f32, const PatchReduce *reduce)
 {
-    const int target_wgs = p->tune.patch_target;
     const int maxL = p->tile_max_layers;
     const size_t wo = (size_t)group * (size_t)(maxL + 2) + (size_t)layer;
-    const int64_t w0 = (layer >= 2 && layer <= maxL) ? p->patch_work_off[wo] : 0, w1 = (layer >= 2 && layer <= maxL) ? p->patch_work_off[wo + 1] : 0;
+    const bool solves = layer >= 2 && layer <= maxL && p->patch_work_off[wo + 1] > p->patch_work_off[wo];
     PatchArgs pa;
     if (reduce) {
         pa.red = *reduce;
         size_reduce(pa.red, npair, native_lg(p, f32), p->patch_NT);
     }
-    if (w1 <= w0 && pa.red.nred == 0) return VRT_OK;
+    if (!solves && pa.red.nred == 0) return VRT_OK;
     pa.ta = ta;
     pa.npair = npair;
     pa.layer = layer;
@@ -1393,42 +1526,22 @@
     pa.quad = (f32 && pa.lgB >= 1 && p->patch_K == 1 && p->tune.patch_quad != 0 && (npair & 1) == 0) ? 1 : 0;
     if (pa.quad) Q = 1;
     pa.lean = (p->tune.patch_lean != 0 && p->patch_K == 1 && Q == 1 && !pa.quad && npair >= 2) ? 1 : 0;
-    const int lgS = pa.lgB - pa.quad;
     pa.Q = Q;
-    pa.nsplit = 1;
-    pa.ngrp = 1 << lgS;
-    if (w1 > w0) {
-        const int64_t items = (w1 - w0) << lgS;
-        const int nblock = pair_block_count(npair, pa.lgB);
-        const int steps_all = (nblock + Q - 1) / Q;
-        int nsplit;
-        if (p->tune.patch_split > 0) nsplit = std::min(steps_all, p->tune.patch_split);
-        else if (target_wgs > 0) nsplit = (int)std::max<int64_t>(1, std::min<int64_t>(steps_all, (target_wgs + items - 1) / items));
-        else {
-            const double T = std::min(900.0, 460.0 + 4100.0 / (double)steps_all);
-            const int s_min = (int)std::min<int64_t>(steps_all, std::max<int64_t>(1, (512 + items - 1) / items));
-            double dmin = 1e300;
-            for (int c = steps_all; c >= 1; c--) {
-                const int sc = (steps_all + c - 1) / c;
-                if (sc >= s_min) dmin = std::min(dmin, std::fabs(std::log((double)items * sc / T)));
-            }
-            nsplit = s_min;
-            for (int c = steps_all; c >= 1; c--) {
-                const int sc = (steps_all + c - 1) / c;
-                if (sc >= s_min && std::fabs(std::log((double)items * sc / T)) <= dmin + 0.03) nsplit = sc;
-            }
-        }
-        pa.nsplit = nsplit;
-        pa.ngrp = nsplit << lgS;
+    int64_t nrec = 0;
+    pa.wrec = nullptr;
+    if (solves) {
+        const vrt_plan::PatchListSet *ls = nullptr;
+        if (int rc = ensure_patch_lists(p, npair, pa.lgB, pa.lgB - pa.quad, Q, ls)) return rc;
+        nrec = ls->off[wo + 1] - ls->off[wo];
+        pa.wrec = ls->recs + 3 * ls->off[wo];
     }
     pa.stride = p->patch_cap + 1;
     pa.cap = p->patch_cap;
     pa.dbg = kDiag ? p->tune.debug_flags : 0;
-    pa.wrec = p->d_patch_work + 2 * w0;
     pa.e_pos = p->e_pos; pa.e_u1 = p->e_u1; pa.e_u2 = p->e_u2;
     pa.e_vis = p->e_vis; pa.e_loc = p->e_loc;
     pa.e_w1 = p->e_w1; pa.e_w2 = p->e_w2; pa.e_r1 = p->e_r1; pa.e_r2 = p->e_r2;
-    const dim3 grid((unsigned)(pa.red.nred + (w1 - w0) * pa.ngrp));
+    const dim3 grid((unsigned)(pa.red.nred + nrec));
     const size_t lds = (size_t)(pa.quad ? 2 : Q) * (size_t)pa.stride * sizeof(double2) + (size_t)pa.cap * (4 * sizeof(double) + 5 * sizeof(int32_t));
     const int rc = f32 ? launch_mode<float>(ta.alpha_mode, p->patch_K, Q, p->patch_NT, grid, lds, st, pa)
                        : launch_mode<double>(ta.alpha_mode, p->patch_K, Q, p->patch_NT, grid, lds, st, pa);
@@ -1504,13 +1617,10 @@
     const int64_t n = g->n, n_patches = p->n_patches;
     const int nblock = pair_block_count(npair, lgB);
     if ((int64_t)nsplit * n_patches >= ((int64_t)1 << 31)) return fail(VRT_EINVAL, "too many (split, patch) progress words");
-    PatchArgs sp;
-    sp.nsplit = nsplit;
-    sp.Q = 1;
     std::vector<int> steps((size_t)nsplit);
     for (int s = 0; s < nsplit; s++) {
         int b0, b1;
-        split_blocks(sp, s, nblock, b0, b1);
+        split_steps(nblock, nsplit, s, b0, b1);
         steps[(size_t)s] = b1 - b0;
     }
     std::vector<int4> q[8];
```

After: 89.31 billion (median of 6 runs). 1.01x the previous value.
